# Peilun-Tommy-Li/pHNN-MPC

Hardware: AMD Instinct MI355X
Metric: pHNN-MPC rollouts+grads/sec, cartpole H=50 batch=65536 (higher is better)
Workload: dtype f32

## Files before the change

### phnn_mpc_amd/csrc/phnn_kernels.hip.h

```cpp
#pragma once
#include <hip/hip_runtime.h>

#include <type_traits>

#include "../../include/phnn_mpc.h"

#define DEV __device__ __forceinline__
#ifdef PHNN_CACHED_TAPE
#define PHNN_NT_STORE(v, p) (*(p) = (v))
#define PHNN_NT_LOAD(p) (*(p))
#else
#define PHNN_NT_STORE(v, p) __builtin_nontemporal_store((v), (p))
#define PHNN_NT_LOAD(p) __builtin_nontemporal_load((p))
#endif

using f32x4 = __attribute__((ext_vector_type(4))) float;
using f32x2 = __attribute__((ext_vector_type(2))) float;

constexpr int kTileB = 16;
#ifndef PHNN_KMAXWAVES
#define PHNN_KMAXWAVES 8
#endif
constexpr int kMaxWaves = PHNN_KMAXWAVES;
constexpr int kScrFloats = 16 * 20;

struct Lane {
  int lane, i, q;
  int w;
  float* xch;
};

template <int T>
struct Act {
  f32x4 v[T];
};

DEV f32x4 mfma(float a, float b, f32x4 c) { return __builtin_amdgcn_mfma_f32_16x16x4f32(a, b, c, 0, 0, 0); }

DEV f32x4 splat4(float s) { return f32x4{s, s, s, s}; }

DEV f32x4 fma4(f32x4 a, f32x4 b, f32x4 c) { return __builtin_elementwise_fma(a, b, c); }
DEV f32x4 dtanh(f32x4 a) { return __builtin_elementwise_fma(-a, a, f32x4{1.0f, 1.0f, 1.0f, 1.0f}); }

DEV float sel4(f32x4 v, int q) { return q == 0 ? v[0] : (q == 1 ? v[1] : (q == 2 ? v[2] : v[3])); }

DEV float tanh_scaled(float x, float c) {
  float e = __builtin_amdgcn_exp2f(x * c);
  return __builtin_fmaf(-2.0f, __builtin_amdgcn_rcpf(e + 1.0f), 1.0f);
}

template <bool ACCURATE>
DEV float tanh_dev(float x) {
  if (ACCURATE) {
    float ax = __builtin_fabsf(x);
    float s = x * x;
    float p = -0.007265716325491667f;
    p = __builtin_fmaf(p, s, 0.021598778665065765f);
    p = __builtin_fmaf(p, s, -0.053949106484651566f);
    p = __builtin_fmaf(p, s, 0.13333284854888916f);
    p = __builtin_fmaf(p, s, -0.3333333432674408f);
    float small = __builtin_fmaf(ax * s, p, ax);
    float e = __builtin_amdgcn_exp2f(ax * 2.8853900817779268f);
    float big = __builtin_fmaf(-2.0f, __builtin_amdgcn_rcpf(e + 1.0f), 1.0f);
    float r = ax < 0.4f ? small : big;
    return __builtin_copysignf(r, x);
  }
  float e = __builtin_amdgcn_exp2f(x * 2.8853900817779268f);
  return __builtin_fmaf(-2.0f, __builtin_amdgcn_rcpf(e + 1.0f), 1.0f);
}

DEV void sincos_dev(float x, float& sn, float& cs) {
  float k = __builtin_rintf(x * 0.6366197723675814f);
  float r = __builtin_fmaf(k, -1.5707963705062866f, x);
  r = __builtin_fmaf(k, 4.371138828673793e-08f, r);
  r = __builtin_fmaf(k, 1.7763568394002505e-15f, r);
  float r2 = r * r;
  float p = 2.723737452470232e-06f;
  p = __builtin_fmaf(p, r2, -0.00019839986634906381f);
  p = __builtin_fmaf(p, r2, 0.008333331905305386f);
  p = __builtin_fmaf(p, r2, -0.1666666716337204f);
  float s0 = __builtin_fmaf(r * r2, p, r);
  float q = -2.721424721130461e-07f;
  q = __builtin_fmaf(q, r2, 2.479966133250855e-05f);
  q = __builtin_fmaf(q, r2, -0.0013888884568586946f);
  q = __builtin_fmaf(q, r2, 0.0416666679084301f);
  float c0 = __builtin_fmaf(r2 * r2, q, __builtin_fmaf(-0.5f, r2, 1.0f));
  int n = (int)k;
  float ss = (n & 1) ? c0 : s0;
  float cc = (n & 1) ? s0 : c0;
  sn = (n & 2) ? -ss : ss;
  cs = ((n + 1) & 2) ? -cc : cc;
}

DEV void keep_lds_reads_local() { asm volatile("" ::: "memory"); }

template <int T>
DEV void tanh_act(Act<T>& a) {
  constexpr bool ACCURATE = T <= 4;
#pragma unroll
  for (int t = 0; t < T; ++t)
#pragma unroll
    for (int r = 0; r < 4; ++r) a.v[t][r] = tanh_dev<ACCURATE>(a.v[t][r]);
}

template <int T>
constexpr bool kPreScaled = T > 4;

template <int T>
DEV void tanh_act_pre(Act<T>& a) {
#pragma unroll
  for (int t = 0; t < T; ++t)
#pragma unroll
    for (int r = 0; r < 4; ++r) {
      if (kPreScaled<T>) a.v[t][r] = __builtin_fmaf(-2.0f, __builtin_amdgcn_rcpf(__builtin_amdgcn_exp2f(a.v[t][r]) + 1.0f), 1.0f);
      else a.v[t][r] = tanh_dev<true>(a.v[t][r]);
    }
}

template <int T>
DEV void load_vec(Act<T>& o, const float* vec, Lane ln) {
  keep_lds_reads_local();
#pragma unroll
  for (int t = 0; t < T; ++t) o.v[t] = *reinterpret_cast<const f32x4*>(vec + 16 * t + 4 * ln.q);
}

template <int T>
DEV void zero_act(Act<T>& o) {
#pragma unroll
  for (int t = 0; t < T; ++t) o.v[t] = splat4(0.f);
}

template <int T>
DEV void in_layer(Act<T>& o, const float* Wf, Lane ln, float xk) {
  keep_lds_reads_local();
#pragma unroll
  for (int nt = 0; nt < T; ++nt) o.v[nt] = mfma(Wf[nt * 64 + ln.lane], xk, o.v[nt]);
}

template <int TO, int TI>
DEV void sq_fwd(Act<TO>& o, const float* W, Lane ln, const Act<TI>& in) {
  constexpr int LD = 16 * TI + 4;
  keep_lds_reads_local();
  const float* base = W + ln.i * LD + 4 * ln.q;
  if (TO == 1) {
    f32x4 e = o.v[0], d = splat4(0.f);
#pragma unroll
    for (int t = 0; t < TI; ++t) {
      f32x4 a = *reinterpret_cast<const f32x4*>(base + 16 * t);
      e = mfma(a[0], in.v[t][0], e);
      d = mfma(a[1], in.v[t][1], d);
      e = mfma(a[2], in.v[t][2], e);
      d = mfma(a[3], in.v[t][3], d);
    }
    o.v[0] = e + d;
    return;
  }
  constexpr int G = TO < 4 ? TO : 4;
#pragma unroll
  for (int t = 0; t < TI; ++t) {
#pragma unroll
    for (int n0 = 0; n0 < TO; n0 += G) {
      f32x4 a[G];
#pragma unroll
      for (int g = 0; g < G; ++g) a[g] = *reinterpret_cast<const f32x4*>(base + (n0 + g) * 16 * LD + 16 * t);
#pragma unroll
      for (int r = 0; r < 4; ++r)
#pragma unroll
        for (int g = 0; g < G; ++g) o.v[n0 + g] = mfma(a[g][r], in.v[t][r], o.v[n0 + g]);
    }
  }
}

template <int TO, int TI>
DEV void sq_bwd(Act<TO>& o, const float* W, Lane ln, const Act<TI>& in) {
  constexpr int LD = 16 * TO + 4;
  keep_lds_reads_local();
  const float* base = W + 4 * ln.q * LD + ln.i;
#pragma unroll
  for (int t = 0; t < TI; ++t)
#pragma unroll
    for (int r = 0; r < 4; ++r)
#pragma unroll
      for (int nt = 0; nt < TO; ++nt) o.v[nt] = mfma(base[(16 * t + r) * LD + 16 * nt], in.v[t][r], o.v[nt]);
}

constexpr int MM_F32 = 0, MM_BF16X3 = 1, MM_F16X2 = 2;
using bf16x2 = __attribute__((ext_vector_type(2))) __bf16;
using bf16x4 = __attribute__((ext_vector_type(4))) __bf16;
using bf16x8 = __attribute__((ext_vector_type(8))) __bf16;
using u32x4 = __attribute__((ext_vector_type(4))) unsigned;

DEV f32x4 mfma_bf(bf16x8 a, bf16x8 b, f32x4 c) { return __builtin_amdgcn_mfma_f32_16x16x32_bf16(a, b, c, 0, 0, 0); }

DEV unsigned pk_bf16(float a, float b) {
  f32x2 v = {a, b};
  return __builtin_bit_cast(unsigned, __builtin_convertvector(v, bf16x2));
}

DEV void matrix_phase_begin() {
#if !defined(PHNN_NO_SETPRIO) && !defined(PHNN_STATIC_PRIO)
  __builtin_amdgcn_s_setprio(0);
#endif
}
DEV void matrix_phase_end() {
#if !defined(PHNN_NO_SETPRIO) && !defined(PHNN_STATIC_PRIO)
  __builtin_amdgcn_s_setprio(2);
#endif
}
DEV void static_prio(int wave) {
#ifdef PHNN_STATIC_PRIO
  if (wave >= 4) __builtin_amdgcn_s_setprio(1);
#endif
}

template <int T>
struct Split3 {
  bf16x8 h[T / 2], m[T / 2], l[T / 2];
};

template <int T>
DEV void split_act(const Act<T>& a, Split3<T>& o) {
#pragma unroll
  for (int s = 0; s < T / 2; ++s) {
    u32x4 H, M, Lo;
#pragma unroll
    for (int p = 0; p < 4; ++p) {
      float x0 = a.v[2 * s + (p >> 1)][2 * (p & 1)], x1 = a.v[2 * s + (p >> 1)][2 * (p & 1) + 1];
      unsigned hb = pk_bf16(x0, x1);
      float r0 = x0 - __builtin_bit_cast(float, hb << 16), r1 = x1 - __builtin_bit_cast(float, hb & 0xffff0000u);
      unsigned mb = pk_bf16(r0, r1);
      float t0 = r0 - __builtin_bit_cast(float, mb << 16), t1 = r1 - __builtin_bit_cast(float, mb & 0xffff0000u);
      H[p] = hb;
      M[p] = mb;
      Lo[p] = pk_bf16(t0, t1);
    }
    o.h[s] = __builtin_bit_cast(bf16x8, H);
    o.m[s] = __builtin_bit_cast(bf16x8, M);
    o.l[s] = __builtin_bit_cast(bf16x8, Lo);
  }
}

template <int HID>
struct BfImg {
  static constexpr int RS = HID + 16;
  static constexpr int PART = HID * RS * 2;
  static constexpr int FLOATS = 3 * PART / 4;
};

DEV void mfma6x2(f32x4& o0, f32x4& o1, const bf16x8 (&a)[2][3], bf16x8 xh, bf16x8 xm, bf16x8 xl) {
  o0 = mfma_bf(a[0][2], xh, o0);
  o1 = mfma_bf(a[1][2], xh, o1);
  o0 = mfma_bf(a[0][0], xl, o0);
  o1 = mfma_bf(a[1][0], xl, o1);
  o0 = mfma_bf(a[0][1], xm, o0);
  o1 = mfma_bf(a[1][1], xm, o1);
  o0 = mfma_bf(a[0][1], xh, o0);
  o1 = mfma_bf(a[1][1], xh, o1);
  o0 = mfma_bf(a[0][0], xm, o0);
  o1 = mfma_bf(a[1][0], xm, o1);
  o0 = mfma_bf(a[0][0], xh, o0);
  o1 = mfma_bf(a[1][0], xh, o1);
}

template <int T>
DEV void sq_fwd_bf(Act<T>& o, const float* Wimg, Lane ln, const Split3<T>& in) {
  using I = BfImg<16 * T>;
  keep_lds_reads_local();
  matrix_phase_begin();
  const char* base = reinterpret_cast<const char*>(Wimg) + ln.i * (I::RS * 2) + ln.q * 16;
#ifdef PHNN_PREFETCH_BF
  {
    bf16x8 a[2][2][3];
    auto loadg = [&](int g, bf16x8 (&dst)[2][3]) {
      const int n0 = 2 * (g / (T / 2)), s = g % (T / 2);
#pragma unroll
      for (int gg = 0; gg < 2; ++gg)
#pragma unroll
        for (int p = 0; p < 3; ++p)
          dst[gg][p] = *reinterpret_cast<const bf16x8*>(base + p * I::PART + (n0 + gg) * 16 * (I::RS * 2) + s * 64);
    };
    constexpr int NG = (T / 2) * (T / 2);
    loadg(0, a[0]);
#pragma unroll
    for (int g = 0; g < NG; ++g) {
      if (g + 1 < NG) loadg(g + 1, a[(g + 1) & 1]);
      __builtin_amdgcn_sched_barrier(0);
      const int n0 = 2 * (g / (T / 2)), s = g % (T / 2);
      mfma6x2(o.v[n0], o.v[n0 + 1], a[g & 1], in.h[s], in.m[s], in.l[s]);
      __builtin_amdgcn_sched_barrier(0);
    }
    matrix_phase_end();
    return;
  }
#endif
#pragma unroll
  for (int n0 = 0; n0 < T; n0 += 2) {
#pragma unroll
    for (int s = 0; s < T / 2; ++s) {
      bf16x8 a[2][3];
#pragma unroll
      for (int g = 0; g < 2; ++g)
#pragma unroll
        for (int p = 0; p < 3; ++p)
          a[g][p] = *reinterpret_cast<const bf16x8*>(base + p * I::PART + (n0 + g) * 16 * (I::RS * 2) + s * 64);
      mfma6x2(o.v[n0], o.v[n0 + 1], a, in.h[s], in.m[s], in.l[s]);
    }
  }
  matrix_phase_end();
}

template <int T>
DEV void sq_bwd_bf(Act<T>& o, const float* Wimg, Lane ln, const Split3<T>& in) {
  using I = BfImg<16 * T>;
  keep_lds_reads_local();
  matrix_phase_begin();
  typedef bf16x4 __attribute__((address_space(3))) * lds_bf4;
  typedef char __attribute__((address_space(3))) * lds_cp;
  const int a4 = (ln.lane & 15) >> 2, pp = ln.lane & 3;
  lds_cp base = (lds_cp) const_cast<char*>(reinterpret_cast<const char*>(Wimg)) + (4 * ln.q + a4) * (I::RS * 2) + 16 * pp;
#ifdef PHNN_PREFETCH_BF
  {
    bf16x8 a[2][2][3];
    auto loadg = [&](int g, bf16x8 (&dst)[2][3]) {
      const int n0 = 2 * (g / (T / 2)), s = g % (T / 2);
#pragma unroll
      for (int gg = 0; gg < 2; ++gg) {
        const int nt = n0 + gg;
#pragma unroll
        for (int p = 0; p < 3; ++p) {
          lds_cp off = base + p * I::PART + 32 * s * (I::RS * 2) + (64 * (nt >> 1) + 8 * (nt & 1));
          bf16x4 lo = __builtin_amdgcn_ds_read_tr16_b64_v4bf16((lds_bf4)off);
          bf16x4 hi = __builtin_amdgcn_ds_read_tr16_b64_v4bf16((lds_bf4)(off + 16 * (I::RS * 2)));
          dst[gg][p] = __builtin_shufflevector(lo, hi, 0, 1, 2, 3, 4, 5, 6, 7);
        }
      }
    };
    constexpr int NG = (T / 2) * (T / 2);
    loadg(0, a[0]);
#pragma unroll
    for (int g = 0; g < NG; ++g) {
      if (g + 1 < NG) loadg(g + 1, a[(g + 1) & 1]);
      __builtin_amdgcn_sched_barrier(0);
      const int n0 = 2 * (g / (T / 2)), s = g % (T / 2);
      mfma6x2(o.v[n0], o.v[n0 + 1], a[g & 1], in.h[s], in.m[s], in.l[s]);
      __builtin_amdgcn_sched_barrier(0);
    }
    matrix_phase_end();
    return;
  }
#endif
#pragma unroll
  for (int n0 = 0; n0 < T; n0 += 2) {
#pragma unroll
    for (int s = 0; s < T / 2; ++s) {
      bf16x8 a[2][3];
#pragma unroll
      for (int g = 0; g < 2; ++g) {
        const int nt = n0 + g;
#pragma unroll
        for (int p = 0; p < 3; ++p) {
          lds_cp off = base + p * I::PART + 32 * s * (I::RS * 2) + (64 * (nt >> 1) + 8 * (nt & 1));
          bf16x4 lo = __builtin_amdgcn_ds_read_tr16_b64_v4bf16((lds_bf4)off);
          bf16x4 hi = __builtin_amdgcn_ds_read_tr16_b64_v4bf16((lds_bf4)(off + 16 * (I::RS * 2)));
          a[g][p] = __builtin_shufflevector(lo, hi, 0, 1, 2, 3, 4, 5, 6, 7);
        }
      }
      mfma6x2(o.v[n0], o.v[n0 + 1], a, in.h[s], in.m[s], in.l[s]);
    }
  }
  matrix_phase_end();
}

using f16x2 = __attribute__((ext_vector_type(2))) _Float16;
using f16x4 = __attribute__((ext_vector_type(4))) _Float16;
using f16x8 = __attribute__((ext_vector_type(8))) _Float16;
typedef __fp16 fp16x4_t __attribute__((__vector_size__(4 * sizeof(__fp16))));

DEV f32x4 mfma_h(f16x8 a, f16x8 b, f32x4 c) { return __builtin_amdgcn_mfma_f32_16x16x32_f16(a, b, c, 0, 0, 0); }

DEV f32x2 residual_h(f16x2 h, f32x2 x) {
#ifdef PHNN_NO_FMAMIX
  return x - __builtin_convertvector(h, f32x2);
#endif
  unsigned hb = __builtin_bit_cast(unsigned, h);
  f32x2 r;
  asm("v_fma_mix_f32 %0, %1, -1.0, %2 op_sel_hi:[1,0,0]" : "=v"(r[0]) : "v"(hb), "v"(x[0]));
  asm("v_fma_mix_f32 %0, %1, -1.0, %2 op_sel:[1,0,0] op_sel_hi:[1,0,0]" : "=v"(r[1]) : "v"(hb), "v"(x[1]));
  return r;
}

template <int T>
struct Split2 {
  f16x8 h[T / 2], l[T / 2];
};

template <int T>
DEV void split_act_h(const Act<T>& a, Split2<T>& o) {
#pragma unroll
  for (int s = 0; s < T / 2; ++s) {
    u32x4 H, Lo;
#pragma unroll
    for (int p = 0; p < 4; ++p) {
      f32x2 x = {a.v[2 * s + (p >> 1)][2 * (p & 1)], a.v[2 * s + (p >> 1)][2 * (p & 1) + 1]};
      f16x2 hb = __builtin_convertvector(x, f16x2);
      f32x2 r = residual_h(hb, x);
      H[p] = __builtin_bit_cast(unsigned, hb);
      Lo[p] = __builtin_bit_cast(unsigned, __builtin_convertvector(r, f16x2));
    }
    o.h[s] = __builtin_bit_cast(f16x8, H);
    o.l[s] = __builtin_bit_cast(f16x8, Lo);
  }
}

template <int HID>
struct HfImg {
  static constexpr int RS = HID + 16;
  static constexpr int PART = HID * RS * 2;
  static constexpr int FLOATS = 2 * PART / 4;
};

DEV f16x8 in_frag_h(f32x4 x) {
// ... 250 lines not shown
  u32x4 H = __builtin_bit_cast(u32x4, o.h[P]), Lo = __builtin_bit_cast(u32x4, o.l[P]);
  H[j] = __builtin_bit_cast(unsigned, hb);
  Lo[j] = __builtin_bit_cast(unsigned, __builtin_convertvector(r, f16x2));
  o.h[P] = __builtin_bit_cast(f16x8, H);
  o.l[P] = __builtin_bit_cast(f16x8, Lo);
}
template <int TI>
struct To4Pairs {
  static_assert(TI >= 2 && TI % 2 == 0, "pairs of tiles");
  const float* row;
  f32x4 tot, o0, o1, a;
  DEV To4Pairs(const float* Wt, Lane ln) : row(Wt + (ln.i & 3) * (16 * TI + 8) + 4 * ln.q) {
    a = *reinterpret_cast<const f32x4*>(row);
  }
  DEV void put(int P, int j, float x0, float x1) {
    const int t = 2 * P + (j >> 1), e = 2 * (j & 1);
    if (j == 0) o0 = o1 = splat4(0.f);
    o0 = __builtin_amdgcn_mfma_f32_4x4x1f32(a[e], x0, o0, 0, 0, 0);
    o1 = __builtin_amdgcn_mfma_f32_4x4x1f32(a[e + 1], x1, o1, 0, 0, 0);
    if (e == 2 && t + 1 < TI) a = *reinterpret_cast<const f32x4*>(row + 16 * (t + 1));
    if (j == 3) tot = P == 0 ? o0 + o1 : tot + (o0 + o1);
  }
  DEV f32x4 finish() const { return to4_kslots(tot); }
};

template <int T>
DEV void store_act(float* dst, Lane ln, const Act<T>& a) {
#pragma unroll
  for (int t = 0; t < T; ++t) PHNN_NT_STORE(a.v[t], reinterpret_cast<f32x4*>(dst) + t * 64 + ln.lane);
}
template <int T>
DEV void load_act(const float* src, Lane ln, Act<T>& a) {
#pragma unroll
  for (int t = 0; t < T; ++t) {
#ifdef PHNN_PLAIN_STASH_LOADS
    a.v[t] = reinterpret_cast<const f32x4*>(src)[t * 64 + ln.lane];
#else
    a.v[t] = PHNN_NT_LOAD(reinterpret_cast<const f32x4*>(src) + t * 64 + ln.lane);
#endif
  }
}

constexpr float kFix24 = 8388607.0f;
typedef unsigned u32x3 __attribute__((ext_vector_type(3), aligned(4)));
template <int T>
DEV void store_act24(float* dst, Lane ln, const Act<T>& a) {
#pragma unroll
  for (int t = 0; t < T; ++t) {
    unsigned q[4];
#pragma unroll
    for (int r = 0; r < 4; ++r) q[r] = (unsigned)(int)__builtin_rintf(a.v[t][r] * kFix24);
    u32x3 d = {__builtin_amdgcn_perm(q[1], q[0], 0x04020100u),
               __builtin_amdgcn_perm(q[2], q[1], 0x05040201u),
               __builtin_amdgcn_perm(q[3], q[2], 0x06050402u)};
    PHNN_NT_STORE(d, reinterpret_cast<u32x3*>(reinterpret_cast<char*>(dst) + (t * 64 + ln.lane) * 12));
  }
}
template <int T>
DEV void load_act24(const float* src, Lane ln, Act<T>& a) {
#pragma unroll
  for (int t = 0; t < T; ++t) {
    const u32x3 d = PHNN_NT_LOAD(reinterpret_cast<const u32x3*>(reinterpret_cast<const char*>(src) + (t * 64 + ln.lane) * 12));
    const int q0 = (int)(d[0] << 8) >> 8;
    const int q1 = (int)(__builtin_amdgcn_alignbit(d[1], d[0], 24) << 8) >> 8;
    const int q2 = (int)(__builtin_amdgcn_alignbit(d[2], d[1], 16) << 8) >> 8;
    const int q3 = (int)d[2] >> 8;
    a.v[t] = f32x4{(float)q0, (float)q1, (float)q2, (float)q3} * (1.0f / kFix24);
  }
}

DEV void gather16(float* scr, Lane ln, f32x4 mine, float (&out)[16]) {
  float* row = scr + ln.i * 20;
  *reinterpret_cast<f32x4*>(row + 4 * ln.q) = mine;
  __builtin_amdgcn_wave_barrier();
#pragma unroll
  for (int k = 0; k < 4; ++k) {
    f32x4 v = *reinterpret_cast<const f32x4*>(row + 4 * k);
    out[4 * k + 0] = v[0];
    out[4 * k + 1] = v[1];
    out[4 * k + 2] = v[2];
    out[4 * k + 3] = v[3];
  }
  __builtin_amdgcn_wave_barrier();
}

DEV float reduce_q(float v) {
#ifdef PHNN_BPERMUTE_REDUCE
  v += __shfl_xor(v, 16);
  v += __shfl_xor(v, 32);
  return v;
#else
  float b;
  asm volatile("v_mov_b32 %1, %0\n\ts_nop 1\n\tv_permlane16_swap_b32 %0, %1\n\ts_nop 0" : "+v"(v), "=&v"(b));
  v += b;
  asm volatile("v_mov_b32 %1, %0\n\ts_nop 1\n\tv_permlane32_swap_b32 %0, %1\n\ts_nop 0" : "+v"(v), "=&v"(b));
  return v + b;
#endif
}


template <int HID, int MM = MM_F32>
struct LayH2 {
  static constexpr int T = HID / 16, LD = HID + 4, LR = HID + 8;
  static constexpr int oW2 = 0;
  static constexpr int W2F = MM == MM_F32 ? HID * LD : (MM == MM_BF16X3 ? BfImg<HID>::FLOATS : HfImg<HID>::FLOATS);
  static constexpr int oW1h = oW2 + W2F;
  static constexpr int oW1f = oW1h + (MM == MM_F16X2 ? T * 64 * 4 : 0);
  static constexpr int oB1 = oW1f + T * 64;
  static constexpr int oB2 = oB1 + HID;
  static constexpr int oW3 = oB2 + HID;
  static constexpr int oW3B = oW3 + HID;
  static constexpr int oW3S = oW3B + HID;
  static constexpr int oW1T = oW3S + HID;
  static constexpr int oB3 = oW1T + 4 * LR;
  static constexpr int SIZE = oB3 + 4;
};

template <int HID, int MM = MM_F32>
struct LayH1 {
  static constexpr int T = HID / 16, LD = HID + 4, LR = HID + 8;
  static constexpr bool HF = MM == MM_F16X2;
  static constexpr int RS = HID + 16;
  static constexpr int FPART = 16 * RS * 2;
  static constexpr int BPART = HID * 16 * 2;
  static constexpr int oV2 = 0;
  static constexpr int oV2T = oV2 + 2 * FPART / 4;
  static constexpr int V2F = HF ? (2 * FPART + 2 * BPART) / 4 : 16 * LD;
  static constexpr int oV1h = oV2 + V2F;
  static constexpr int oV1f = oV1h + (HF ? T * 64 * 4 : 0);
  static constexpr int oC1 = oV1f + T * 64;
  static constexpr int oC2 = oC1 + HID;
  static constexpr int oSc = oC2 + 16;
  static constexpr int oV1T = oSc + 4;
  static constexpr int SIZE = oV1T + 4 * LR;
};

constexpr int kRecSmall = 40;
template <int T, int NBIG>
struct WRec {
  static constexpr int VEC = T * 256;
  static constexpr int oSmall = NBIG * VEC;
  static constexpr int SIZE = oSmall + 16 * kRecSmall;
};

#ifdef PHNN_CACHED_RECORDS
#define PHNN_REC_STORE(v, p) (*(p) = (v))
#define PHNN_REC_LOAD(p) (*(p))
#else
#define PHNN_REC_STORE(v, p) __builtin_nontemporal_store((v), (p))
#define PHNN_REC_LOAD(p) __builtin_nontemporal_load((p))
#endif
template <int T>
DEV void store_rec(float* dst, Lane ln, const Act<T>& a) {
#pragma unroll
  for (int t = 0; t < T; ++t) PHNN_REC_STORE(a.v[t], reinterpret_cast<f32x4*>(dst) + t * 64 + ln.lane);
}
template <int T>
DEV void store_rec_scaled(float* dst, Lane ln, const Act<T>& a, float s) {
#pragma unroll
  for (int t = 0; t < T; ++t) PHNN_REC_STORE(a.v[t] * s, reinterpret_cast<f32x4*>(dst) + t * 64 + ln.lane);
}

constexpr int ACT_TANH = 0, ACT_SILU = 2, ACT_RELU = 3, ACT_ELU = 4, ACT_GELU = 5;

DEV float gelu_pdf(float z) { return 0.3989422804014327f * __builtin_amdgcn_exp2f(z * z * -0.7213475204444817f); }
DEV float gelu_cdf(float z) { return __builtin_fmaf(0.5f, erff(z * 0.7071067811865476f), 0.5f); }

template <int ACT>
DEV void act_eval(float z, float& a, float& d1) {
  if (ACT == ACT_RELU) {
    a = fmaxf(z, 0.f);
    d1 = z > 0.f ? 1.0f : 0.0f;
  } else if (ACT == ACT_ELU) {
    a = z > 0.f ? z : expm1f(z);
    d1 = z > 0.f ? 1.0f : __builtin_amdgcn_exp2f(z * 1.4426950408889634f);
  } else if (ACT == ACT_GELU) {
    const float c = gelu_cdf(z);
    a = z * c;
    d1 = __builtin_fmaf(z, gelu_pdf(z), c);
  } else {
    const float s = __builtin_amdgcn_rcpf(1.0f + __builtin_amdgcn_exp2f(z * -1.4426950408889634f));
    a = z * s;
    d1 = __builtin_fmaf(a, 1.0f - s, s);
  }
}
template <int ACT>
DEV float act_d2(float z) {
  if (ACT == ACT_RELU) return 0.0f;
  if (ACT == ACT_ELU) return z > 0.f ? 0.0f : __builtin_amdgcn_exp2f(z * 1.4426950408889634f);
  if (ACT == ACT_GELU) return gelu_pdf(z) * fmaxf(__builtin_fmaf(-z, z, 2.0f), -3.0e38f);
  const float s = __builtin_amdgcn_rcpf(1.0f + __builtin_amdgcn_exp2f(z * -1.4426950408889634f));
  return s * (1.0f - s) * __builtin_fmaf(z, 1.0f - 2.0f * s, 2.0f);
}
template <int ACT, int T>
DEV void act_of(const Act<T>& z, Act<T>& a) {
#pragma unroll
  for (int t = 0; t < T; ++t)
#pragma unroll
    for (int r = 0; r < 4; ++r) {
      float av, d;
      act_eval<ACT>(z.v[t][r], av, d);
      a.v[t][r] = av;
    }
}
template <int ACT, int T>
DEV void mul_d1(Act<T>& g, const Act<T>& z) {
#pragma unroll
  for (int t = 0; t < T; ++t)
#pragma unroll
    for (int r = 0; r < 4; ++r) {
      float a, d;
      act_eval<ACT>(z.v[t][r], a, d);
      g.v[t][r] *= d;
    }
}

constexpr int TAPE_NONE = 0, TAPE_MPC = 1, TAPE_TRAIN = 2;
template <class M, int TK>
constexpr int tape_floats() {
  if constexpr (TK == TAPE_MPC && M::CURV) return M::TAPE_C;
  else return M::STASH;
}

template <int HID>
struct HTape {
  Act<HID / 16> a1, a2, q1;
};

template <int HID, bool WANT_H, int ACT>
DEV f32x4 hnet_grad_g(const float* L, Lane ln, f32x4 x, HTape<HID>& tp, float& Hval) {
  using Y = LayH2<HID, MM_F32>;
  constexpr int T = Y::T;
  load_vec<T>(tp.a1, L + Y::oB1, ln);
  in_layer<T>(tp.a1, L + Y::oW1f, ln, sel4(x, ln.q));
  {
    Act<T> a;
    act_of<ACT, T>(tp.a1, a);
    load_vec<T>(tp.a2, L + Y::oB2, ln);
    sq_fwd<T, T>(tp.a2, L + Y::oW2, ln, a);
  }
  Act<T> g;
  float s = 0.f;
  keep_lds_reads_local();
#pragma unroll
  for (int t = 0; t < T; ++t) {
    f32x4 w3 = *reinterpret_cast<const f32x4*>(L + Y::oW3 + 16 * t + 4 * ln.q);
#pragma unroll
    for (int r = 0; r < 4; ++r) {
      float a, d;
      act_eval<ACT>(tp.a2.v[t][r], a, d);
      if (WANT_H) s = __builtin_fmaf(w3[r], a, s);
      g.v[t][r] = w3[r] * d;
    }
  }
  if (WANT_H) Hval = reduce_q(s) + L[Y::oB3];
  zero_act<T>(tp.q1);
  sq_bwd<T, T>(tp.q1, L + Y::oW2, ln, g);
#pragma unroll
  for (int t = 0; t < T; ++t) g.v[t] = tp.q1.v[t];
  mul_d1<ACT, T>(g, tp.a1);
  return to4_rep<T>(L + Y::oW1T, ln, g);
}
template <int HID, int ACT>
DEV void hnet_layer1_g(const float* L, Lane ln, f32x4 x, Act<HID / 16>& z1) {
  using Y = LayH2<HID, MM_F32>;
  load_vec<Y::T>(z1, L + Y::oB1, ln);
  in_layer<Y::T>(z1, L + Y::oW1f, ln, sel4(x, ln.q));
}
template <int HID, int ACT>
DEV f32x4 hnet_hvp_g(const float* L, Lane ln, HTape<HID>& tp, f32x4 v) {
  using Y = LayH2<HID, MM_F32>;
  constexpr int T = Y::T;
  Act<T> ad1, w;
  zero_act<T>(ad1);
  in_layer<T>(ad1, L + Y::oW1f, ln, sel4(v, ln.q));
#pragma unroll
  for (int t = 0; t < T; ++t)
#pragma unroll
    for (int r = 0; r < 4; ++r) {
      const float z = tp.a1.v[t][r], zd = ad1.v[t][r];
      float a, d;
      act_eval<ACT>(z, a, d);
      tp.q1.v[t][r] = tp.q1.v[t][r] * (act_d2<ACT>(z) * zd);
      ad1.v[t][r] = d * zd;
    }
  zero_act<T>(w);
  sq_fwd<T, T>(w, L + Y::oW2, ln, ad1);
  keep_lds_reads_local();
#pragma unroll
  for (int t = 0; t < T; ++t) {
    f32x4 w3 = *reinterpret_cast<const f32x4*>(L + Y::oW3 + 16 * t + 4 * ln.q);
#pragma unroll
    for (int r = 0; r < 4; ++r) w.v[t][r] = w3[r] * (act_d2<ACT>(tp.a2.v[t][r]) * w.v[t][r]);
  }
  Act<T> qd;
  zero_act<T>(qd);
  sq_bwd<T, T>(qd, L + Y::oW2, ln, w);
  mul_d1<ACT, T>(qd, tp.a1);
#pragma unroll
  for (int t = 0; t < T; ++t) qd.v[t] = qd.v[t] + tp.q1.v[t];
  return to4_rep<T>(L + Y::oW1T, ln, qd);
}

template <int HID, bool WANT_H, int MM = MM_F32, int SITE = kInHFwd, int ACT = ACT_TANH, int FE = 0>
DEV f32x4 hnet_grad(const float* L, Lane ln, f32x4 z, HTape<HID>& tp, float& Hval) {
  if constexpr (ACT != ACT_TANH) {
    static_assert(MM == MM_F32, "SiLU / ReLU run on the all-f32 kernels");
    return hnet_grad_g<HID, WANT_H, ACT>(L, ln, z, tp, Hval);
  }
  using Y = LayH2<HID, MM>;
  constexpr int T = Y::T;
  load_vec<T>(tp.a1, L + Y::oB1, ln);
  in_layer_mm<T, MM, SITE>(tp.a1, L, Y::oW1f, Y::oW1h, ln, z);
  tanh_act_pre<T>(tp.a1);
  load_vec<T>(tp.a2, L + Y::oB2, ln);
  constexpr bool FUSABLE = MM == MM_F16X2 && SITE == kInHFwd && T >= 2 && T % 2 == 0;
  constexpr bool FUSE_ACT = FUSABLE && (FE & kFuseSites & kFuseK1Act) != 0, FUSE_RED = FUSABLE && (FE & kFuseSites & kFuseK1Red) != 0;
  Split2<T> spg{};
  float s = 0.f;
  if constexpr (FUSE_ACT) {
    Split2<T> sp;
    split_act_h<T>(tp.a1, sp);
    const float c = L[Y::oB3 + 1];
    f32x4 w3 = splat4(0.f), w3b = *reinterpret_cast<const f32x4*>(L + Y::oW3B + 4 * ln.q);
    if (WANT_H) w3 = *reinterpret_cast<const f32x4*>(L + Y::oW3 + 4 * ln.q);
    auto act = [&](auto pre) {
      return [&](int P, int j) {
        const int t = 2 * P + (j >> 1), e = 2 * (j & 1);
        f32x2 g;
#pragma unroll
        for (int k = 0; k < 2; ++k) {
          const float x = tp.a2.v[t][e + k];
          const float a = decltype(pre)::value ? __builtin_fmaf(-2.0f, __builtin_amdgcn_rcpf(__builtin_amdgcn_exp2f(x) + 1.0f), 1.0f)
                                               : tanh_scaled(x, c);
          tp.a2.v[t][e + k] = a;
          if (WANT_H) s = __builtin_fmaf(w3[e + k], a, s);
          g[k] = w3b[e + k] * __builtin_fmaf(-a, a, 1.0f);
        }
        if (e == 2 && t + 1 < T) {
          if (WANT_H) w3 = *reinterpret_cast<const f32x4*>(L + Y::oW3 + 16 * (t + 1) + 4 * ln.q);
          w3b = *reinterpret_cast<const f32x4*>(L + Y::oW3B + 16 * (t + 1) + 4 * ln.q);
        }
        split_put_h<T>(spg, P, j, g);
      };
    };
    if (kPreScaled<T> && c == 1.0f) sq_fwd_h<T>(tp.a2, L + Y::oW2, ln, sp, act(std::true_type()));
    else sq_fwd_h<T>(tp.a2, L + Y::oW2, ln, sp, act(std::false_type()));
  } else if (MM == MM_BF16X3) {
    Split3<T> sp;
    split_act<T>(tp.a1, sp);
    sq_fwd_bf<T>(tp.a2, L + Y::oW2, ln, sp);
  } else if (MM == MM_F16X2) {
    Split2<T> sp;
    split_act_h<T>(tp.a1, sp);
    sq_fwd_h<T>(tp.a2, L + Y::oW2, ln, sp);
  } else {
    sq_fwd<T, T>(tp.a2, L + Y::oW2, ln, tp.a1);
  }
  if constexpr (FUSE_ACT) {
  } else if (MM == MM_F16X2 || kPreScaled<T>) {
    const float c = L[Y::oB3 + 1];
    if (kPreScaled<T> && c == 1.0f) {
      tanh_act_pre<T>(tp.a2);
    } else {
#pragma unroll
      for (int t = 0; t < T; ++t)
#pragma unroll
        for (int r = 0; r < 4; ++r) tp.a2.v[t][r] = tanh_scaled(tp.a2.v[t][r], c);
    }
  } else {
    tanh_act<T>(tp.a2);
  }
  Act<T> g;
  keep_lds_reads_local();
  if constexpr (!FUSE_ACT) {
#pragma unroll
    for (int t = 0; t < T; ++t) {
      if (WANT_H) {
        f32x4 w3 = *reinterpret_cast<const f32x4*>(L + Y::oW3 + 16 * t + 4 * ln.q);
#pragma unroll
        for (int r = 0; r < 4; ++r) s = __builtin_fmaf(w3[r], tp.a2.v[t][r], s);
      }
      f32x4 w3b = *reinterpret_cast<const f32x4*>(L + Y::oW3B + 16 * t + 4 * ln.q);
      g.v[t] = w3b * dtanh(tp.a2.v[t]);
    }
  }
  if (WANT_H) Hval = reduce_q(s) + L[Y::oB3];
  zero_act<T>(tp.q1);
  if constexpr (FUSABLE) {
    if constexpr (!FUSE_ACT) split_act_h<T>(g, spg);
    if constexpr (FUSE_RED) {
      To4Pairs<T> red(L + Y::oW1T, ln);
      sq_bwd_h<T>(tp.q1, L + Y::oW2, ln, spg, [&](int P, int j) {
        const int t = 2 * P + (j >> 1), e = 2 * (j & 1);
        const float a0 = tp.a1.v[t][e], a1 = tp.a1.v[t][e + 1];
        red.put(P, j, tp.q1.v[t][e] * __builtin_fmaf(-a0, a0, 1.0f), tp.q1.v[t][e + 1] * __builtin_fmaf(-a1, a1, 1.0f));
      });
      return red.finish();
    } else {
      sq_bwd_h<T>(tp.q1, L + Y::oW2, ln, spg);
    }
  } else if (MM == MM_BF16X3) {
    Split3<T> sp;
    split_act<T>(g, sp);
    sq_bwd_bf<T>(tp.q1, L + Y::oW2, ln, sp);
  } else if (MM == MM_F16X2) {
    Split2<T> sp;
    split_act_h<T>(g, sp);
    sq_bwd_h<T>(tp.q1, L + Y::oW2, ln, sp);
  } else {
    sq_bwd<T, T>(tp.q1, L + Y::oW2, ln, g);
  }
#pragma unroll
  for (int t = 0; t < T; ++t) g.v[t] = tp.q1.v[t] * dtanh(tp.a1.v[t]);
  return to4_rep<T>(L + Y::oW1T, ln, g);
}

template <int HID, int MM, int ACT = ACT_TANH>
DEV void hnet_layer1(const float* L, Lane ln, f32x4 z, Act<HID / 16>& a1) {
  if constexpr (ACT != ACT_TANH) return hnet_layer1_g<HID, ACT>(L, ln, z, a1);
  using Y = LayH2<HID, MM>;
  load_vec<Y::T>(a1, L + Y::oB1, ln);
  in_layer_mm<Y::T, MM, kInHRecomp>(a1, L, Y::oW1f, Y::oW1h, ln, z);
  tanh_act_pre<Y::T>(a1);
}

template <int HID>
struct CurvImg {
  static constexpr int RS = HID + 16, PART = 10 * RS * 2;
  static constexpr int oConst = 2 * PART / 4;
  static constexpr int FLOATS = oConst + 4;
};
struct Curv {
  float m[16];
};
template <int T>
DEV void hnet_curv_operand(const Act<T>& q1, const Act<T>& a1, Split2<T>& sp) {
  Act<T> c;
#pragma unroll
  for (int t = 0; t < T; ++t) c.v[t] = (q1.v[t] * dtanh(a1.v[t])) * a1.v[t];
  split_act_h<T>(c, sp);
}
template <int HID>
DEV f32x4 hnet_curv_kstep(const float* P, Lane ln, int s, f16x8 ch, f16x8 cl) {
  using I = CurvImg<HID>;
  keep_lds_reads_local();
  const int a = ln.i >> 2, b = ln.i & 3, lo = a < b ? a : b, hi = a < b ? b : a;
  const int row = (lo * (9 - lo)) / 2 + (hi - lo);
  const char* base = reinterpret_cast<const char*>(P) + row * (I::RS * 2) + ln.q * 16 + s * 64;
  const f16x8 ah = *reinterpret_cast<const f16x8*>(base);
  const f16x8 al = *reinterpret_cast<const f16x8*>(base + I::PART);
  return mfma_h(ah, ch, mfma_h(ah, cl, mfma_h(al, ch, splat4(0.f))));
}
template <int HID>
DEV f32x4 hnet_curv(const float* P, Lane ln, const HTape<HID>& tp) {
  constexpr int T = HID / 16;
  Split2<T> sp;
  hnet_curv_operand<T>(tp.q1, tp.a1, sp);
  f32x4 tot = hnet_curv_kstep<HID>(P, ln, 0, sp.h[0], sp.l[0]);
#pragma unroll
  for (int s = 1; s < T / 2; ++s) tot = tot + hnet_curv_kstep<HID>(P, ln, s, sp.h[s], sp.l[s]);
  return tot * P[CurvImg<HID>::oConst];
}
DEV void spread_curv(f32x4 mine, Lane ln, Curv& c) {
#pragma unroll
  for (int r = 0; r < 4; ++r)
#pragma unroll
    for (int j = 0; j < 4; ++j) c.m[4 * r + j] = __shfl(mine[j], 16 * r + ln.i);
}
DEV f32x4 curv_apply(const Curv& c, f32x4 v) {
  f32x4 o;
#pragma unroll
  for (int r = 0; r < 4; ++r) {
    float s = 0.f;
#pragma unroll
    for (int j = 0; j < 4; ++j) s = __builtin_fmaf(c.m[4 * r + j], v[j], s);
    o[r] = s;
  }
  return o;
}

template <int HID, bool COMPACT>
DEV void hnet_tape_store(float* stash, int oC, const float* P, Lane ln, const HTape<HID>& tp, f32x4 dH) {
  constexpr int T = HID / 16;
  store_act<T>(stash, ln, tp.a2);
  if constexpr (COMPACT) {
    if (ln.q == 0) PHNN_NT_STORE(dH, reinterpret_cast<f32x4*>(stash + T * 256) + ln.i);
    PHNN_NT_STORE(hnet_curv<HID>(P, ln, tp), reinterpret_cast<f32x4*>(stash + oC) + ln.i * 4 + ln.q);
  } else {
    store_act<T>(stash + T * 256, ln, tp.q1);
    if (ln.q == 0) PHNN_NT_STORE(dH, reinterpret_cast<f32x4*>(stash + 2 * T * 256) + ln.i);
  }
}
template <int T, bool COMPACT>
DEV f32x4 tape_load_dH(const float* stash, Lane ln) {
  return PHNN_NT_LOAD(reinterpret_cast<const f32x4*>(stash + (COMPACT ? 1 : 2) * T * 256) + ln.i);
}
DEV void load_curv(const float* src, Lane ln, Curv& c) {
  const f32x4* p = reinterpret_cast<const f32x4*>(src) + ln.i * 4;
#pragma unroll
  for (int k = 0; k < 4; ++k) {
    f32x4 v = PHNN_NT_LOAD(p + k);
#pragma unroll
    for (int e = 0; e < 4; ++e) c.m[4 * k + e] = v[e];
  }
}
template <int HID, bool COMPACT>
DEV void hnet_tape_load(const float* stash, int oC, Lane ln, HTape<HID>& tp, Curv& cv) {
  constexpr int T = HID / 16;
  load_act<T>(stash, ln, tp.a2);
  if constexpr (COMPACT) load_curv(stash + oC, ln, cv);
  else load_act<T>(stash + T * 256, ln, tp.q1);
}

template <int HID, int MM = MM_F32, bool WG = false, int ACT = ACT_TANH, int SITE = kInHHvp, bool CQ = false, int FE = 0>
DEV f32x4 hnet_hvp(const float* L, Lane ln, HTape<HID>& tp, f32x4 v, float* rec = nullptr, const Curv* cv = nullptr) {
  static_assert(!CQ || (MM == MM_F16X2 && ACT == ACT_TANH && !WG), "the curvature block exists for f16x2 Tanh MPC kernels");
  if constexpr (ACT != ACT_TANH) {
    static_assert(!WG, "weight-gradient kernels exist for Tanh models only");
    return hnet_hvp_g<HID, ACT>(L, ln, tp, v);
  }
  using Y = LayH2<HID, MM>;
  constexpr int T = Y::T;
  float unscale = 1.0f;
  if (MM == MM_F16X2) {
    float mx = fmaxf(fmaxf(__builtin_fabsf(v[0]), __builtin_fabsf(v[1])), fmaxf(__builtin_fabsf(v[2]), __builtin_fabsf(v[3])));
    int e = 0;
    (void)__builtin_frexpf(mx, &e);
    e = (mx > 0.f && mx < 3.0e38f) ? e : 0;
    v = v * __builtin_ldexpf(1.0f, -e);
    unscale = __builtin_ldexpf(1.0f, e);
  }
  Act<T> ad1, w;
  zero_act<T>(ad1);
  in_layer_mm<T, MM, SITE>(ad1, L, Y::oW1f, Y::oW1h, ln, v);
#pragma unroll
  for (int t = 0; t < T; ++t) ad1.v[t] = dtanh(tp.a1.v[t]) * ad1.v[t];
  if constexpr (!CQ) {
#pragma unroll
    for (int t = 0; t < T; ++t) tp.q1.v[t] = tp.q1.v[t] * (tp.a1.v[t] * ad1.v[t]);
  }
  zero_act<T>(w);
  constexpr bool FUSABLE = CQ && T >= 2 && T % 2 == 0;
  constexpr bool FUSE_ACT = FUSABLE && (FE & kFuseSites & kFuseK2Act) != 0, FUSE_RED = FUSABLE && (FE & kFuseSites & kFuseK2Red) != 0;
  Split2<T> spw{};
  if constexpr (FUSE_ACT) {
    Split2<T> sp;
    split_act_h<T>(ad1, sp);
    f32x4 w3 = *reinterpret_cast<const f32x4*>(L + Y::oW3S + 4 * ln.q);
    sq_fwd_h<T>(w, L + Y::oW2, ln, sp, [&](int P, int j) {
      const int t = 2 * P + (j >> 1), e = 2 * (j & 1);
      f32x2 x;
#pragma unroll
      for (int k = 0; k < 2; ++k) {
        const float a2 = tp.a2.v[t][e + k];
        const float ad2 = __builtin_fmaf(-a2, a2, 1.0f) * w.v[t][e + k];
        x[k] = w3[e + k] * (a2 * ad2);
      }
      if (e == 2 && t + 1 < T) w3 = *reinterpret_cast<const f32x4*>(L + Y::oW3S + 16 * (t + 1) + 4 * ln.q);
      split_put_h<T>(spw, P, j, x);
    });
  } else {
    if (MM == MM_BF16X3) {
      Split3<T> sp;
      split_act<T>(ad1, sp);
      sq_fwd_bf<T>(w, L + Y::oW2, ln, sp);
    } else if (MM == MM_F16X2) {
      Split2<T> sp;
      split_act_h<T>(ad1, sp);
      sq_fwd_h<T>(w, L + Y::oW2, ln, sp);
    } else {
      sq_fwd<T, T>(w, L + Y::oW2, ln, ad1);
    }
    keep_lds_reads_local();
#pragma unroll
    for (int t = 0; t < T; ++t) {
      f32x4 w3 = *reinterpret_cast<const f32x4*>(L + Y::oW3S + 16 * t + 4 * ln.q);
      f32x4 a2 = tp.a2.v[t];
      f32x4 ad2 = dtanh(a2) * w.v[t];
      if (WG) PHNN_REC_STORE(ad2 * unscale, reinterpret_cast<f32x4*>(rec + 2 * T * 256) + t * 64 + ln.lane);
      w.v[t] = w3 * (a2 * ad2);
    }
  }
  Act<T> qd;
  zero_act<T>(qd);
  if constexpr (FUSABLE) {
    if constexpr (!FUSE_ACT) split_act_h<T>(w, spw);
    if constexpr (FUSE_RED) {
      To4Pairs<T> red(L + Y::oW1T, ln);
      sq_bwd_h<T>(qd, L + Y::oW2, ln, spw, [&](int P, int j) {
        const int t = 2 * P + (j >> 1), e = 2 * (j & 1);
        const float a0 = tp.a1.v[t][e], a1 = tp.a1.v[t][e + 1];
        red.put(P, j, qd.v[t][e] * __builtin_fmaf(-a0, a0, 1.0f), qd.v[t][e + 1] * __builtin_fmaf(-a1, a1, 1.0f));
      });
      return (red.finish() * (-2.0f * L[Y::oB3 + 2]) + curv_apply(*cv, v)) * unscale;
    } else {
      sq_bwd_h<T>(qd, L + Y::oW2, ln, spw);
    }
  } else if (MM == MM_BF16X3) {
    Split3<T> sp;
    split_act<T>(w, sp);
    sq_bwd_bf<T>(qd, L + Y::oW2, ln, sp);
  } else if (MM == MM_F16X2) {
    Split2<T> sp;
    split_act_h<T>(w, sp);
    sq_bwd_h<T>(qd, L + Y::oW2, ln, sp);
  } else {
    sq_bwd<T, T>(qd, L + Y::oW2, ln, w);
  }
  if (WG) store_rec_scaled<T>(rec + 3 * T * 256, ln, qd, unscale);
#pragma unroll
  for (int t = 0; t < T; ++t) {
    if constexpr (CQ) qd.v[t] = qd.v[t] * dtanh(tp.a1.v[t]);
    else qd.v[t] = __builtin_elementwise_fma(qd.v[t], dtanh(tp.a1.v[t]), tp.q1.v[t]);
  }
  f32x4 Hv = to4_rep<T>(L + Y::oW1T, ln, qd);
  if constexpr (CQ) return (Hv * (-2.0f * L[Y::oB3 + 2]) + curv_apply(*cv, v)) * unscale;
  return Hv * (-2.0f * unscale * L[Y::oB3 + 2]);
}

template <int HID, int MM>
DEV f32x4 h1_out_hf(const float* L, Lane ln, const Split2<HID / 16>& sp) {
  using Y = LayH1<HID, MM>;
  constexpr int T = Y::T;
  keep_lds_reads_local();
  const char* base = reinterpret_cast<const char*>(L + Y::oV2) + ln.i * (Y::RS * 2) + ln.q * 16;
  f32x4 o0 = splat4(0.f), o1 = splat4(0.f), o2 = splat4(0.f);
#pragma unroll
  for (int s = 0; s < T / 2; ++s) {
    f16x8 ah = *reinterpret_cast<const f16x8*>(base + s * 64);
    f16x8 al = *reinterpret_cast<const f16x8*>(base + Y::FPART + s * 64);
    o0 = mfma_h(al, sp.h[s], o0);
    o1 = mfma_h(ah, sp.l[s], o1);
    o2 = mfma_h(ah, sp.h[s], o2);
  }
  const float inv = L[Y::oSc];
  f32x4 c2 = *reinterpret_cast<const f32x4*>(L + Y::oC2 + 4 * ln.q);
  return ((o0 + o1) + o2) * inv + c2;
}

template <int HID, int MM>
DEV void h1_bwd_operands(const float* L, Lane ln, const float (&obar)[16], f16x8& b1, f16x8& b2, float& unscale) {
  using Y = LayH1<HID, MM>;
  float mx = 0.f;
#pragma unroll
  for (int k = 0; k < 16; ++k) mx = fmaxf(mx, __builtin_fabsf(obar[k]));
  int e = 0;
  (void)__builtin_frexpf(mx, &e);
  e = (mx > 0.f && mx < 3.0e38f) ? e : 0;
  const float sc = __builtin_ldexpf(1.0f, -e);
  unscale = __builtin_ldexpf(1.0f, e) * L[Y::oSc];
  const bool second = (ln.q & 1) != 0, lo_half = ln.q >= 2;
  u32x4 B1, B2;
#pragma unroll
  for (int p = 0; p < 4; ++p) {
    f32x2 v = {(second ? obar[8 + 2 * p] : obar[2 * p]) * sc, (second ? obar[9 + 2 * p] : obar[2 * p + 1]) * sc};
    f16x2 hb2 = __builtin_convertvector(v, f16x2);
    f32x2 r = residual_h(hb2, v);
    unsigned hbits = __builtin_bit_cast(unsigned, hb2), lbits = __builtin_bit_cast(unsigned, __builtin_convertvector(r, f16x2));
    B1[p] = lo_half ? lbits : hbits;
    B2[p] = lo_half ? 0u : hbits;
  }
  b1 = __builtin_bit_cast(f16x8, B1);
  b2 = __builtin_bit_cast(f16x8, B2);
}

DEV void store_rf(float* dst, Lane ln, f32x4 o) {
  if (ln.w == 0) PHNN_NT_STORE(o, reinterpret_cast<f32x4*>(dst) + ln.i * 4 + ln.q);
}
DEV void load_rf(const float* src, Lane ln, float (&rf)[16]) {
  const f32x4* p = reinterpret_cast<const f32x4*>(src) + ln.i * 4;
#pragma unroll
  for (int k = 0; k < 4; ++k) {
    f32x4 v = PHNN_NT_LOAD(p + k);
#pragma unroll
    for (int e = 0; e < 4; ++e) rf[4 * k + e] = v[e];
  }
}
template <int HID, int MM = MM_F32, int SITE = kInHNet1, int ACT = ACT_TANH>
DEV void h1_hidden(const float* L, Lane ln, f32x4 x, Act<HID / 16>& h) {
  using Y = LayH1<HID, MM>;
  constexpr int T = Y::T;
  load_vec<T>(h, L + Y::oC1, ln);
  in_layer_mm<T, MM, SITE>(h, L, Y::oV1f, Y::oV1h, ln, x);
  if constexpr (ACT == ACT_TANH) tanh_act_pre<T>(h);
}

template <int HID, int MM = MM_F32, int SITE = kInHNet1, int ACT = ACT_TANH>
DEV void h1_fwd(const float* L, float* scr, Lane ln, f32x4 x, Act<HID / 16>& h, float (&out)[16], float* rf_stash = nullptr) {
  using Y = LayH1<HID, MM>;
  constexpr int T = Y::T;
  load_vec<T>(h, L + Y::oC1, ln);
  in_layer_mm<T, MM, SITE>(h, L, Y::oV1f, Y::oV1h, ln, x);
  if constexpr (ACT != ACT_TANH) {
    static_assert(MM == MM_F32, "SiLU / ReLU run on the all-f32 kernels");
    Act<T> a;
    act_of<ACT, T>(h, a);
    Act<1> og;
    og.v[0] = *reinterpret_cast<const f32x4*>(L + Y::oC2 + 4 * ln.q);
    sq_fwd<1, T>(og, L + Y::oV2, ln, a);
    if (rf_stash) store_rf(rf_stash, ln, og.v[0]);
    gather16(scr, ln, og.v[0], out);
    return;
  }
  tanh_act_pre<T>(h);
  Act<1> o;
  if (Y::HF) {
    Split2<T> sp;
    split_act_h<T>(h, sp);
    o.v[0] = h1_out_hf<HID, MM>(L, ln, sp);
  } else {
    o.v[0] = *reinterpret_cast<const f32x4*>(L + Y::oC2 + 4 * ln.q);
    sq_fwd<1, T>(o, L + Y::oV2, ln, h);
  }
  if (rf_stash) store_rf(rf_stash, ln, o.v[0]);
  gather16(scr, ln, o.v[0], out);
}

template <int HID, int MM = MM_F32, bool WG = false, int ACT = ACT_TANH>
DEV f32x4 h1_bwd(const float* L, Lane ln, const Act<HID / 16>& h, const float (&obar)[16], float* rec = nullptr) {
  using Y = LayH1<HID, MM>;
  constexpr int T = Y::T;
  Act<T> hb;
  if constexpr (ACT != ACT_TANH) {
    static_assert(MM == MM_F32 && !WG, "SiLU / ReLU: all-f32 kernels, no weight-gradient records");
    Act<1> ob;
#pragma unroll
    for (int r = 0; r < 4; ++r)
      ob.v[0][r] = ln.q == 0 ? obar[r] : (ln.q == 1 ? obar[4 + r] : (ln.q == 2 ? obar[8 + r] : obar[12 + r]));
    zero_act<T>(hb);
    sq_bwd<T, 1>(hb, L + Y::oV2, ln, ob);
    mul_d1<ACT, T>(hb, h);
    return to4_rep<T>(L + Y::oV1T, ln, hb);
  }
  float unscale = 1.0f;
  if (Y::HF) {
    f16x8 b1, b2;
    h1_bwd_operands<HID, MM>(L, ln, obar, b1, b2, unscale);
    keep_lds_reads_local();
    const char* base = reinterpret_cast<const char*>(L + Y::oV2T) + ln.i * 32 + (ln.q & 1) * 16;
#pragma unroll
    for (int nt = 0; nt < T; ++nt) {
      f16x8 ah = *reinterpret_cast<const f16x8*>(base + nt * 512);
      f16x8 al = *reinterpret_cast<const f16x8*>(base + Y::BPART + nt * 512);
      hb.v[nt] = mfma_h(ah, b1, mfma_h(al, b2, splat4(0.f)));
    }
  } else {
    Act<1> ob;
#pragma unroll
    for (int r = 0; r < 4; ++r)
      ob.v[0][r] = ln.q == 0 ? obar[r] : (ln.q == 1 ? obar[4 + r] : (ln.q == 2 ? obar[8 + r] : obar[12 + r]));
    zero_act<T>(hb);
    sq_bwd<T, 1>(hb, L + Y::oV2, ln, ob);
  }
#pragma unroll
  for (int t = 0; t < T; ++t) hb.v[t] = hb.v[t] * dtanh(h.v[t]);
  if (WG) store_rec_scaled<T>(rec, ln, hb, Y::HF ? unscale : 1.0f);
  f32x4 xb = to4_rep<T>(L + Y::oV1T, ln, hb);
  return Y::HF ? xb * unscale : xb;
}

template <int N>
DEV void sym_from_rf(const float (&rf)[16], float (&S)[N][N]) {
#pragma unroll
  for (int i = 0; i < N; ++i) {
    S[i][i] = rf[i * N + i];
#pragma unroll
    for (int j = i + 1; j < N; ++j) S[i][j] = S[j][i] = (rf[i * N + j] + rf[j * N + i]) * 0.5f;
  }
}
template <int N>
DEV void rbar_from(f32x4 lam, f32x4 dH, const float (&Stl)[N], const float (&StdH)[N], float (&rbar)[16]) {
  float m[N][N];
#pragma unroll
  for (int k = 0; k < 16; ++k) rbar[k] = 0.f;
#pragma unroll
  for (int i = 0; i < N; ++i)
#pragma unroll
    for (int j = 0; j < N; ++j) m[i][j] = __builtin_fmaf(lam[i], StdH[j], dH[i] * Stl[j]);
#pragma unroll
  for (int i = 0; i < N; ++i) {
    rbar[i * N + i] = -m[i][i];
#pragma unroll
    for (int j = i + 1; j < N; ++j) rbar[i * N + j] = rbar[j * N + i] = (m[i][j] + m[j][i]) * -0.5f;
  }
}

template <int N_, int HID_, bool FIXG_, int MM_ = MM_F32, int MI_ = 1, int ACT_ = ACT_TANH>
struct PhnnModel {
  static constexpr int N = N_, HID = HID_, T = HID / 16, MM = MM_, MI = MI_, ACT = ACT_;
  static constexpr bool FIXG = FIXG_, SPLIT = false;
  static_assert(N_ * MI_ <= 16 && MI_ <= 4, "G_net output n*m <= 16, m <= 4");
  static constexpr int SCR = kScrFloats;
  static constexpr int oH = 0;
  static constexpr int oR = oH + LayH2<HID, MM>::SIZE;
  static constexpr int oGn = oR + LayH1<HID, MM>::SIZE;
  static constexpr int oJ = oGn + (FIXG ? 0 : LayH1<HID, MM>::SIZE);
  static constexpr int oG = oJ + 16;
  static constexpr int oP = oG + 16;
  static constexpr bool CURV = MM == MM_F16X2 && ACT == ACT_TANH &&
                               4 * (oP + CurvImg<HID>::FLOATS + kMaxWaves * SCR) <= 160 * 1024;
  static constexpr int IMG = oP + (CURV ? CurvImg<HID>::FLOATS : 0);
  static constexpr int FUSE = (HID_ != 128 || !FIXG_) ? 0 : ((MI_ <= 2 ? PHNN_FUSE_K1 : 0) | (MI_ == 1 ? PHNN_FUSE_K2 : 0));

  static constexpr int oStashRf = 2 * T * 256 + 64;
  static constexpr int STASH = oStashRf + 256;
  static constexpr int oTapeRf = T * 256 + 64, oTapeC = oTapeRf + 256, TAPE_C = oTapeC + 256;

  template <bool WANT_H, int TK = TAPE_NONE, int FE = 0>
  DEV static f32x4 f(const float* L, float* scr, Lane ln, f32x4 x, f32x4 u, float& Hval, float* stash = nullptr) {
    constexpr bool ST = TK != TAPE_NONE, CT = TK == TAPE_MPC && CURV;
    keep_lds_reads_local();
    HTape<HID> tp;
    f32x4 dH = hnet_grad<HID, WANT_H, MM, kInHFwd, ACT, FE>(L + oH, ln, x, tp, Hval);
    if (ST) hnet_tape_store<HID, CT>(stash, oTapeC, L + oP, ln, tp, dH);
    Act<T> hR;
    float rf[16];
    h1_fwd<HID, MM, kInHNet1, ACT>(L + oR, scr, ln, x, hR, rf, ST ? stash + (CT ? oTapeRf : oStashRf) : nullptr);
    float G[N * MI];
    if (FIXG) {
#pragma unroll
      for (int i = 0; i < N * MI; ++i) G[i] = L[oG + i];
    } else {
      Act<T> hG;
      float gf[16];
      h1_fwd<HID, MM, kInHNet1, ACT>(L + oGn, scr, ln, x, hG, gf);
#pragma unroll
      for (int i = 0; i < N * MI; ++i) G[i] = gf[i];
    }
    return combine(L, rf, dH, G, u);
  }

  DEV static f32x4 combine(const float* L, const float (&rf)[16], f32x4 dH, const float (&G)[N * MI], f32x4 u) {
    float S[N][N], StdH[N];
    sym_from_rf<N>(rf, S);
#pragma unroll
    for (int k = 0; k < N; ++k) {
      float a = 0.f;
#pragma unroll
      for (int i = 0; i < N; ++i) a = __builtin_fmaf(S[i][k], dH[i], a);
      StdH[k] = a;
    }
    f32x4 dx = splat4(0.f);
#pragma unroll
    for (int i = 0; i < N; ++i) {
      float acc = 0.f;
#pragma unroll
      for (int j = 0; j < N; ++j) acc = __builtin_fmaf(L[oJ + i * N + j], dH[j], acc);
#pragma unroll
      for (int k = 0; k < N; ++k) acc = __builtin_fmaf(-S[i][k], StdH[k], acc);
      if (MI == 1) {
        dx[i] = __builtin_fmaf(G[i], u[0], acc);
      } else {
        float gu = 0.f;
#pragma unroll
        for (int k = 0; k < MI; ++k) gu = __builtin_fmaf(G[i * MI + k], u[k], gu);
        dx[i] = acc + gu;
      }
    }
    return dx;
  }

  static constexpr bool RECHB = !LayH1<HID, MM>::HF;
  static constexpr int NBIG = 4 + (RECHB ? (FIXG ? 1 : 2) : 0);
  using Rec = WRec<T, NBIG>;

  template <bool ST = false, bool WG = false, int INH = -1, int FE = 0>
  DEV static void vjp(const float* L, float* scr, Lane ln, f32x4 x, f32x4 u, f32x4 lam, f32x4& xbar, f32x4& ubar,
                      const float* stash = nullptr, float* rec = nullptr, float Hbar = 0.f) {
    constexpr bool CQ = CURV && !WG;
    keep_lds_reads_local();
    HTape<HID> tp;
    Curv cv;
    float Hdummy;
    f32x4 dH;
    float rf[16];
    if (ST) {
      dH = tape_load_dH<T, CQ>(stash, ln);
      load_rf(stash + (CQ ? oTapeRf : oStashRf), ln, rf);
      hnet_tape_load<HID, CQ>(stash, oTapeC, ln, tp, cv);
    } else {
      dH = hnet_grad<HID, false, MM, INH & kInHRecomp, ACT>(L + oH, ln, x, tp, Hdummy);
      if constexpr (CQ) spread_curv(hnet_curv<HID>(L + oP, ln, tp), ln, cv);
    }
    if (WG && !ST) {
      store_rec<T>(rec, ln, tp.a2);
      store_rec<T>(rec + Rec::VEC, ln, tp.q1);
    }
    f32x4 xb = splat4(0.f);
    float S[N][N], Stl[N], StdH[N];
    {
      Act<T> hR;
      if (ST) {
        h1_hidden<HID, MM, INH & kInHNet1Adj, ACT>(L + oR, ln, x, hR);
      } else {
        h1_fwd<HID, MM, INH & kInHNet1Adj, ACT>(L + oR, scr, ln, x, hR, rf);
      }
      sym_from_rf<N>(rf, S);
#pragma unroll
      for (int k = 0; k < N; ++k) {
        float a = 0.f, c = 0.f;
#pragma unroll
        for (int i = 0; i < N; ++i) {
          a = __builtin_fmaf(S[i][k], lam[i], a);
          c = __builtin_fmaf(S[i][k], dH[i], c);
        }
        Stl[k] = a;
        StdH[k] = c;
      }
      float rbar[16];
      rbar_from<N>(lam, dH, Stl, StdH, rbar);
      xb += h1_bwd<HID, MM, WG && RECHB, ACT>(L + oR, ln, hR, rbar, WG && RECHB ? rec + 4 * Rec::VEC : nullptr);
      if (WG && ln.q == 0) {
        f32x4* sm = reinterpret_cast<f32x4*>(rec + Rec::oSmall + ln.i * kRecSmall);
#pragma unroll
        for (int k = 0; k < 4; ++k) sm[4 + k] = f32x4{rbar[4 * k], rbar[4 * k + 1], rbar[4 * k + 2], rbar[4 * k + 3]};
      }
    }
    ubar = splat4(0.f);
    if (FIXG) {
#pragma unroll
      for (int k = 0; k < MI; ++k)
#pragma unroll
        for (int i = 0; i < N; ++i) ubar[k] = __builtin_fmaf(L[oG + i * MI + k], lam[i], ubar[k]);
    } else {
      Act<T> hG;
      float gf[16], gbar[16];
      h1_fwd<HID, MM, INH & kInHNet1Adj, ACT>(L + oGn, scr, ln, x, hG, gf);
#pragma unroll
      for (int k = 0; k < 16; ++k) gbar[k] = 0.f;
#pragma unroll
      for (int i = 0; i < N; ++i)
#pragma unroll
        for (int k = 0; k < MI; ++k) {
          ubar[k] = __builtin_fmaf(gf[i * MI + k], lam[i], ubar[k]);
          gbar[i * MI + k] = lam[i] * u[k];
        }
      xb += h1_bwd<HID, MM, WG && RECHB, ACT>(L + oGn, ln, hG, gbar, WG && RECHB ? rec + 5 * Rec::VEC : nullptr);
    }
    f32x4 v = splat4(0.f);
#pragma unroll
    for (int j = 0; j < N; ++j) {
      float acc = 0.f;
#pragma unroll
      for (int i = 0; i < N; ++i) acc = __builtin_fmaf(L[oJ + i * N + j], lam[i], acc);
#pragma unroll
      for (int k = 0; k < N; ++k) acc = __builtin_fmaf(-S[j][k], Stl[k], acc);
      v[j] = acc;
    }
    if (WG && ln.q == 0) {
      f32x4* sm = reinterpret_cast<f32x4*>(rec + Rec::oSmall + ln.i * kRecSmall);
      sm[0] = x;
      sm[1] = v;
      sm[2] = lam;
      sm[3] = dH;
      sm[8] = u;
      sm[9] = f32x4{Hbar, 0.f, 0.f, 0.f};
    }
    if (ST) hnet_layer1<HID, MM, ACT>(L + oH, ln, x, tp.a1);
    xbar = xb + hnet_hvp<HID, MM, WG, ACT, INH & kInHHvp, CQ, ST ? FE : 0>(L + oH, ln, tp, v, rec, &cv);
    if (WG) xbar = xbar + Hbar * dH;
  }
};

struct LayM {
  static constexpr int HID = 64, T = 4, LD = HID + 4, LR = HID + 8;
  static constexpr int oW1f = 0;
  static constexpr int oB1 = oW1f + T * 64;
  static constexpr int oW2 = oB1 + HID;
  static constexpr int oB2 = oW2 + HID * LD;
  static constexpr int oWo = oB2 + HID;
  static constexpr int oBo = oWo + 4 * LR;
  static constexpr int oWoTf = oBo + 4;
  static constexpr int oW1T = oWoTf + T * 64;
  static constexpr int SIZE = oW1T + 4 * LR;
};

struct MTape {
  Act<4> a1, a2;
  f32x4 o;
};

DEV void mnet_fwd(const float* L, Lane ln, f32x4 q, MTape& tp) {
  using Y = LayM;
  keep_lds_reads_local();
  load_vec<4>(tp.a1, L + Y::oB1, ln);
  in_layer<4>(tp.a1, L + Y::oW1f, ln, sel4(q, ln.q));
  tanh_act<4>(tp.a1);
  load_vec<4>(tp.a2, L + Y::oB2, ln);
  sq_fwd<4, 4>(tp.a2, L + Y::oW2, ln, tp.a1);
  tanh_act<4>(tp.a2);
  tp.o = to4_rep<4>(L + Y::oWo, ln, tp.a2) + *reinterpret_cast<const f32x4*>(L + Y::oBo);
}

DEV f32x4 mnet_bwd(const float* L, Lane ln, const MTape& tp, f32x4 ob) {
  using Y = LayM;
  keep_lds_reads_local();
  Act<4> d, e;
  zero_act<4>(d);
  in_layer<4>(d, L + Y::oWoTf, ln, sel4(ob, ln.q));
#pragma unroll
  for (int t = 0; t < 4; ++t) d.v[t] = d.v[t] * dtanh(tp.a2.v[t]);
  zero_act<4>(e);
  sq_bwd<4, 4>(e, L + Y::oW2, ln, d);
#pragma unroll
  for (int t = 0; t < 4; ++t) e.v[t] = e.v[t] * dtanh(tp.a1.v[t]);
  return to4_rep<4>(L + Y::oW1T, ln, e);
}

DEV float softplus_dev(float x) { return x > 20.f ? x : log1pf(expf(x)); }
DEV float sigmoid_sp_dev(float x) { return x > 20.f ? 1.0f : 1.0f / (1.0f + expf(-x)); }

constexpr int MASS_CARTPOLE = 0, MASS_CONSTANT = 1, MASS_DIAGONAL = 2, MASS_FULL = 3;

template <int MT>
DEV void mass_from_outputs(f32x4 o, float (&m)[3], float (&w)[3]) {
  if (MT == MASS_DIAGONAL) {
    m[0] = expf(o[0]) + 1e-3f;
    m[2] = expf(o[1]) + 1e-3f;
    m[1] = 0.f;
    w[0] = 1.0f / m[0];
    w[2] = 1.0f / m[2];
    w[1] = 0.f;
  } else {
    const float l00 = softplus_dev(o[0]) + 1e-3f, l10 = o[1], l11 = softplus_dev(o[2]) + 1e-3f;
    m[0] = l00 * l00;
    m[1] = l00 * l10;
    m[2] = l10 * l10 + l11 * l11;
    const float det = m[0] * m[2] - m[1] * m[1];
    w[0] = m[2] / det;
    w[1] = -m[1] / det;
    w[2] = m[0] / det;
  }
}

template <int MT>
DEV f32x4 mass_outputs_bar(f32x4 o, const float (&Mb)[4]) {
  if (MT == MASS_DIAGONAL) return f32x4{Mb[0] * expf(o[0]), Mb[3] * expf(o[1]), 0.f, 0.f};
  const float l00 = softplus_dev(o[0]) + 1e-3f, l10 = o[1], l11 = softplus_dev(o[2]) + 1e-3f;
  const float s00 = 2.0f * Mb[0], s01 = Mb[1] + Mb[2], s11 = 2.0f * Mb[3];
  return f32x4{(s00 * l00 + s01 * l10) * sigmoid_sp_dev(o[0]), s01 * l00 + s11 * l10, (s11 * l11) * sigmoid_sp_dev(o[2]), 0.f};
}

template <int HID_, int MM_ = MM_F32, int MI_ = 1, int MT_ = MASS_CARTPOLE, int ACT_ = ACT_TANH>
struct CanonModel {
  static constexpr int N = 4, HID = HID_, T = HID / 16, MM = MM_, MI = MI_, MT = MT_, ACT = ACT_;
  static constexpr bool SPLIT = false;
  static constexpr int SCR = 0;
  static constexpr int oH = 0;
  static constexpr int oC = oH + LayH2<HID, MM>::SIZE;
  static constexpr int oCG = oC + 12;
  static constexpr int oCW = oC + 28;
  static constexpr int oMn = oC + 32;
  static constexpr int oP = oMn + (MT_ >= MASS_DIAGONAL ? LayM::SIZE : 0);
  static constexpr bool CURV = MM_ == MM_F16X2 && ACT_ == ACT_TANH;
  static constexpr int FUSE = (HID_ == 128 && MT_ <= MASS_CONSTANT) ? PHNN_FUSE_K1 : 0;
  static constexpr int IMG = oP + (CURV ? CurvImg<HID>::FLOATS : 0);

  DEV static void mass_eval(const float* L, Lane ln, f32x4 y, float (&m)[3], float (&w)[3], MTape& mt) {
    if (MT == MASS_CONSTANT) {
      m[0] = L[oC + 0]; m[1] = L[oC + 1]; m[2] = L[oC + 2];
      w[0] = L[oCW + 0]; w[1] = L[oCW + 1]; w[2] = L[oCW + 2];
    } else {
      mnet_fwd(L + oMn, ln, f32x4{y[0], y[1], 0.f, 0.f}, mt);
      mass_from_outputs<MT>(mt.o, m, w);
    }
  }

  DEV static float Base_Gu(const float* L, int row, f32x4 u) {
    float s = 0.f;
#pragma unroll
    for (int k = 0; k < MI; ++k) s = __builtin_fmaf(L[oCG + row * MI + k], u[k], s);
    return s;
  }
  DEV static f32x4 Base_Gt(const float* L, float dpb0, float dpb1) {
    f32x4 ub = splat4(0.f);
#pragma unroll
    for (int k = 0; k < MI; ++k) ub[k] = L[oCG + 2 * MI + k] * dpb0 + L[oCG + 3 * MI + k] * dpb1;
    return ub;
  }

  static constexpr int STASH = 2 * T * 256 + 64;
  static constexpr int oTapeC = T * 256 + 64, TAPE_C = oTapeC + 256;

  template <bool WANT_H, int TK = TAPE_NONE, int FE = 0>
  DEV static f32x4 f(const float* L, float* scr, Lane ln, f32x4 y, f32x4 u, float& Hval, float* stash = nullptr) {
    constexpr bool ST = TK != TAPE_NONE, CT = TK == TAPE_MPC && CURV;
    keep_lds_reads_local();
    if constexpr (MT != MASS_CARTPOLE) {
      float m[3], w[3];
      MTape mt;
      mass_eval(L, ln, y, m, w, mt);
      f32x4 z = {y[0], y[1], m[0] * y[2] + m[1] * y[3], m[1] * y[2] + m[2] * y[3]};
      HTape<HID> tp;
      f32x4 dH = hnet_grad<HID, WANT_H, MM, kInHFwd, ACT, FE>(L + oH, ln, z, tp, Hval);
      if (ST) hnet_tape_store<HID, CT>(stash, oTapeC, L + oP, ln, tp, dH);
      float dp0 = (-dH[0] - L[oC + 6] * dH[2]) + Base_Gu(L, 2, u);
      float dp1 = (-dH[1] - L[oC + 7] * dH[3]) + Base_Gu(L, 3, u);
      return f32x4{w[0] * z[2] + w[1] * z[3], w[1] * z[2] + w[2] * z[3], w[0] * dp0 + w[1] * dp1, w[1] * dp0 + w[2] * dp1};
    }
    float a = L[oC + 0], b = L[oC + 1], c = L[oC + 2];
    float sn, cs;
    sincos_dev(y[1], sn, cs);
    float bc = b * cs;
    f32x4 z = {y[0], y[1], a * y[2] + bc * y[3], bc * y[2] + c * y[3]};
    HTape<HID> tp;
    f32x4 dH = hnet_grad<HID, WANT_H, MM, kInHFwd, ACT, FE>(L + oH, ln, z, tp, Hval);
    if (ST) hnet_tape_store<HID, CT>(stash, oTapeC, L + oP, ln, tp, dH);
    float dp0 = (-dH[0] - L[oC + 6] * dH[2]) + Base_Gu(L, 2, u);
    float dp1 = (-dH[1] - L[oC + 7] * dH[3]) + Base_Gu(L, 3, u);
    float det = (a * c - bc * bc) + 1e-6f;
    float mi00 = c / det, mi01 = -bc / det, mi11 = a / det;
    return f32x4{mi00 * z[2] + mi01 * z[3], mi01 * z[2] + mi11 * z[3], mi00 * dp0 + mi01 * dp1,
                 mi01 * dp0 + mi11 * dp1};
  }

  static constexpr int NBIG = 4;
  using Rec = WRec<T, NBIG>;

  template <bool ST = false, bool WG = false, int INH = -1, int FE = 0>
  DEV static void vjp(const float* L, float* scr, Lane ln, f32x4 y, f32x4 u, f32x4 lam, f32x4& ybar, f32x4& ubar,
                      const float* stash = nullptr, float* rec = nullptr, float Hbar = 0.f) {
    constexpr bool CQ = CURV && !WG;
    Curv cv;
    keep_lds_reads_local();
    if constexpr (MT != MASS_CARTPOLE) {
      float m[3], w[3];
      MTape mt;
      mass_eval(L, ln, y, m, w, mt);
      f32x4 z = {y[0], y[1], m[0] * y[2] + m[1] * y[3], m[1] * y[2] + m[2] * y[3]};
      HTape<HID> tp;
      float Hdummy;
      f32x4 dH;
      if (ST) {
        dH = tape_load_dH<T, CQ>(stash, ln);
        hnet_tape_load<HID, CQ>(stash, oTapeC, ln, tp, cv);
        hnet_layer1<HID, MM, ACT>(L + oH, ln, z, tp.a1);
      } else {
        dH = hnet_grad<HID, false, MM, INH & kInHRecomp, ACT>(L + oH, ln, z, tp, Hdummy);
        if constexpr (CQ) spread_curv(hnet_curv<HID>(L + oP, ln, tp), ln, cv);
      }
      const float Rd2 = L[oC + 6], Rd3 = L[oC + 7];
      const float dp0 = (-dH[0] - Rd2 * dH[2]) + Base_Gu(L, 2, u);
      const float dp1 = (-dH[1] - Rd3 * dH[3]) + Base_Gu(L, 3, u);
      const float pb0 = lam[0] * w[0] + lam[1] * w[1], pb1 = lam[0] * w[1] + lam[1] * w[2];
      const float dpb0 = lam[2] * w[0] + lam[3] * w[1], dpb1 = lam[2] * w[1] + lam[3] * w[2];
      f32x4 v = {-dpb0, -dpb1, -Rd2 * dpb0, -Rd3 * dpb1};
      ubar = Base_Gt(L, dpb0, dpb1);
      if (WG) {
        if (!ST) {
          store_rec<T>(rec, ln, tp.a2);
          store_rec<T>(rec + Rec::VEC, ln, tp.q1);
        }
        if (ln.q == 0) {
          f32x4* sm = reinterpret_cast<f32x4*>(rec + Rec::oSmall + ln.i * kRecSmall);
          sm[0] = z;
          sm[1] = v;
          sm[2] = lam;
          sm[3] = dH;
          sm[4] = f32x4{0.f, 0.f, -dpb0 * dH[2], -dpb1 * dH[3]};
          sm[8] = u;
          sm[9] = f32x4{Hbar, 0.f, 0.f, 0.f};
        }
      }
      f32x4 zb = hnet_hvp<HID, MM, WG, ACT, INH & kInHHvp, CQ, ST ? FE : 0>(L + oH, ln, tp, v, rec, &cv);
      if (WG) zb = zb + Hbar * dH;
      zb[2] += pb0;
      zb[3] += pb1;
      ybar = f32x4{zb[0], zb[1], zb[2] * m[0] + zb[3] * m[1], zb[2] * m[1] + zb[3] * m[2]};
      if (MT >= MASS_DIAGONAL || WG) {
        const float W4[4] = {w[0], w[1], w[1], w[2]};
        const float Wb[4] = {lam[0] * z[2] + lam[2] * dp0, lam[0] * z[3] + lam[2] * dp1,
                             lam[1] * z[2] + lam[3] * dp0, lam[1] * z[3] + lam[3] * dp1};
        float Tm[4], Um[4], Mb[4];
        Tm[0] = W4[0] * Wb[0] + W4[1] * Wb[2]; Tm[1] = W4[0] * Wb[1] + W4[1] * Wb[3];
        Tm[2] = W4[2] * Wb[0] + W4[3] * Wb[2]; Tm[3] = W4[2] * Wb[1] + W4[3] * Wb[3];
        Um[0] = Tm[0] * W4[0] + Tm[1] * W4[2]; Um[1] = Tm[0] * W4[1] + Tm[1] * W4[3];
        Um[2] = Tm[2] * W4[0] + Tm[3] * W4[2]; Um[3] = Tm[2] * W4[1] + Tm[3] * W4[3];
        Mb[0] = zb[2] * y[2] - Um[0];
        Mb[1] = zb[2] * y[3] - Um[1];
        Mb[2] = zb[3] * y[2] - Um[2];
        Mb[3] = zb[3] * y[3] - Um[3];
        if (WG && ln.q == 0) {
          f32x4* sm = reinterpret_cast<f32x4*>(rec + Rec::oSmall + ln.i * kRecSmall);
          sm[5] = f32x4{Mb[0], Mb[1], Mb[2], Mb[3]};
          sm[6] = f32x4{y[0], y[1], 0.f, 0.f};
        }
        if (MT >= MASS_DIAGONAL) {
          f32x4 qb = mnet_bwd(L + oMn, ln, mt, mass_outputs_bar<MT>(mt.o, Mb));
          ybar[0] += qb[0];
          ybar[1] += qb[1];
        }
      }
      return;
    }
    float a = L[oC + 0], b = L[oC + 1], c = L[oC + 2];
    float sn, cs;
    sincos_dev(y[1], sn, cs);
    float bc = b * cs;
    f32x4 z = {y[0], y[1], a * y[2] + bc * y[3], bc * y[2] + c * y[3]};
    HTape<HID> tp;
    float Hdummy;
    f32x4 dH;
    if (ST) {
      dH = tape_load_dH<T, CQ>(stash, ln);
      hnet_tape_load<HID, CQ>(stash, oTapeC, ln, tp, cv);
      hnet_layer1<HID, MM, ACT>(L + oH, ln, z, tp.a1);
    } else {
      dH = hnet_grad<HID, false, MM, INH & kInHRecomp, ACT>(L + oH, ln, z, tp, Hdummy);
      if constexpr (CQ) spread_curv(hnet_curv<HID>(L + oP, ln, tp), ln, cv);
    }
    float Rd2 = L[oC + 6], Rd3 = L[oC + 7];
    float dp0 = (-dH[0] - Rd2 * dH[2]) + Base_Gu(L, 2, u);
    float dp1 = (-dH[1] - Rd3 * dH[3]) + Base_Gu(L, 3, u);
    float det = (a * c - bc * bc) + 1e-6f;
    float rdet = 1.0f / det;
    float mi00 = c * rdet, mi01 = -bc * rdet, mi11 = a * rdet;
    float pb0 = lam[0] * mi00 + lam[1] * mi01, pb1 = lam[0] * mi01 + lam[1] * mi11;
    float dpb0 = lam[2] * mi00 + lam[3] * mi01, dpb1 = lam[2] * mi01 + lam[3] * mi11;
    float mb00 = lam[0] * z[2] + lam[2] * dp0;
    float mb01 = lam[0] * z[3] + lam[1] * z[2] + lam[2] * dp1 + lam[3] * dp0;
    float mb11 = lam[1] * z[3] + lam[3] * dp1;
    f32x4 v = {-dpb0, -dpb1, -Rd2 * dpb0, -Rd3 * dpb1};
    ubar = Base_Gt(L, dpb0, dpb1);
    if (WG) {
      if (!ST) {
        store_rec<T>(rec, ln, tp.a2);
        store_rec<T>(rec + Rec::VEC, ln, tp.q1);
      }
      if (ln.q == 0) {
        f32x4* sm = reinterpret_cast<f32x4*>(rec + Rec::oSmall + ln.i * kRecSmall);
        sm[0] = z;
        sm[1] = v;
        sm[2] = lam;
        sm[3] = dH;
        sm[4] = f32x4{0.f, 0.f, -dpb0 * dH[2], -dpb1 * dH[3]};
        sm[8] = u;
        sm[9] = f32x4{Hbar, 0.f, 0.f, 0.f};
      }
    }
    f32x4 zb = hnet_hvp<HID, MM, WG, ACT, INH & kInHHvp, CQ, ST ? FE : 0>(L + oH, ln, tp, v, rec, &cv);
    if (WG) zb = zb + Hbar * dH;
    zb[2] += pb0;
    zb[3] += pb1;
    float bcb = zb[2] * y[3] + zb[3] * y[2];
    float detb = (-(mb00 * c + mb11 * a) + mb01 * bc) * (rdet * rdet);
    bcb += -mb01 * rdet;
    bcb += -2.0f * bc * detb;
    ybar = f32x4{zb[0], zb[1] + bcb * (-b * sn), zb[2] * a + zb[3] * bc, zb[2] * bc + zb[3] * c};
  }
};

constexpr int kXR0 = 0, kXR1 = 2048, kXR2 = 4096, kXP0 = 6144, kXP1 = 7168, kXchFloats = 8192;
using ActW = Act<2>;

DEV void xch_put(float* region, Lane ln, const Split2<2>& sp) {
  f16x8* p = reinterpret_cast<f16x8*>(region);
  p[ln.w * 64 + ln.lane] = sp.h[0];
  p[(4 + ln.w) * 64 + ln.lane] = sp.l[0];
}
DEV void xch_get(const float* region, Lane ln, Split2<8>& o) {
  const f16x8* p = reinterpret_cast<const f16x8*>(region);
#pragma unroll
  for (int s = 0; s < 4; ++s) {
    o.h[s] = p[s * 64 + ln.lane];
    o.l[s] = p[(4 + s) * 64 + ln.lane];
  }
}
DEV void xch_put_partial(float* set, Lane ln, f32x4 v) { reinterpret_cast<f32x4*>(set)[ln.w * 64 + ln.lane] = v; }
DEV f32x4 xch_sum_partials(const float* set, Lane ln) {
  const f32x4* p = reinterpret_cast<const f32x4*>(set) + ln.lane;
  return to4_kslots(((p[0] + p[64]) + p[128]) + p[192]);
}

DEV void tanh_pre_w(ActW& a) {
#pragma unroll
  for (int t = 0; t < 2; ++t)
#pragma unroll
    for (int r = 0; r < 4; ++r) a.v[t][r] = __builtin_fmaf(-2.0f, __builtin_amdgcn_rcpf(__builtin_amdgcn_exp2f(a.v[t][r]) + 1.0f), 1.0f);
}

DEV void sq_fwd_h_w(ActW& o, const float* Wimg, Lane ln, const Split2<8>& in) {
  using I = HfImg<128>;
  keep_lds_reads_local();
  matrix_phase_begin();
  const char* base = reinterpret_cast<const char*>(Wimg) + ln.i * (I::RS * 2) + ln.q * 16 + (2 * ln.w) * 16 * (I::RS * 2);
#pragma unroll
  for (int s = 0; s < 4; ++s) {
    f16x8 a[2][2];
#pragma unroll
    for (int g = 0; g < 2; ++g)
#pragma unroll
      for (int p = 0; p < 2; ++p) a[g][p] = *reinterpret_cast<const f16x8*>(base + p * I::PART + g * 16 * (I::RS * 2) + s * 64);
    mfma3x2(o.v[0], o.v[1], a, in.h[s], in.l[s]);
  }
  matrix_phase_end();
}

DEV void sq_bwd_h_w(ActW& o, const float* Wimg, Lane ln, const Split2<8>& in) {
  using I = HfImg<128>;
  keep_lds_reads_local();
  matrix_phase_begin();
  typedef fp16x4_t __attribute__((address_space(3))) * lds_h4;
  typedef char __attribute__((address_space(3))) * lds_cp;
  const int a4 = (ln.lane & 15) >> 2, pp = ln.lane & 3;
  lds_cp base = (lds_cp) const_cast<char*>(reinterpret_cast<const char*>(Wimg)) + (4 * ln.q + a4) * (I::RS * 2) + 16 * pp + 64 * ln.w;
#pragma unroll
  for (int s = 0; s < 4; ++s) {
    f16x8 a[2][2];
#pragma unroll
    for (int g = 0; g < 2; ++g)
#pragma unroll
      for (int p = 0; p < 2; ++p) {
        lds_cp off = base + p * I::PART + 32 * s * (I::RS * 2) + 8 * g;
        f16x4 lo = __builtin_bit_cast(f16x4, __builtin_amdgcn_ds_read_tr16_b64_v4f16((lds_h4)off));
        f16x4 hi = __builtin_bit_cast(f16x4, __builtin_amdgcn_ds_read_tr16_b64_v4f16((lds_h4)(off + 16 * (I::RS * 2))));
        a[g][p] = __builtin_shufflevector(lo, hi, 0, 1, 2, 3, 4, 5, 6, 7);
      }
    mfma3x2(o.v[0], o.v[1], a, in.h[s], in.l[s]);
  }
  matrix_phase_end();
}

struct HTapeW {
  ActW a1, a2, q1;
};
DEV void curv_put_w(const float* P, Lane ln, const HTapeW& tp) {
  Split2<2> sp;
  hnet_curv_operand<2>(tp.q1, tp.a1, sp);
  xch_put_partial(ln.xch + kXP1, ln, hnet_curv_kstep<128>(P, ln, ln.w, sp.h[0], sp.l[0]));
}
DEV f32x4 curv_get_w(const float* P, Lane ln) {
  const f32x4* p = reinterpret_cast<const f32x4*>(ln.xch + kXP1) + ln.lane;
  return (((p[0] + p[64]) + p[128]) + p[192]) * P[CurvImg<128>::oConst];
}

template <int SITE = kInHFwd, class PreBarrier>
DEV f32x4 hnet_grad_w(const float* L, Lane ln, f32x4 z, HTapeW& tp, PreBarrier pre_barrier) {
  using Y = LayH2<128, MM_F16X2>;
  const int t0 = 2 * ln.w;
  load_vec<2>(tp.a1, L + Y::oB1 + 16 * t0, ln);
  in_layer_mm<2, MM_F16X2, SITE>(tp.a1, L, Y::oW1f, Y::oW1h, ln, z, t0);
  tanh_pre_w(tp.a1);
  {
    Split2<2> sp;
    split_act_h<2>(tp.a1, sp);
    xch_put(ln.xch + kXR0, ln, sp);
  }
  pre_barrier();
  __syncthreads();
  {
    Split2<8> all;
    xch_get(ln.xch + kXR0, ln, all);
    load_vec<2>(tp.a2, L + Y::oB2 + 16 * t0, ln);
    sq_fwd_h_w(tp.a2, L + Y::oW2, ln, all);
  }
  const float c = L[Y::oB3 + 1];
  if (c == 1.0f) {
    tanh_pre_w(tp.a2);
  } else {
#pragma unroll
    for (int t = 0; t < 2; ++t)
#pragma unroll
      for (int r = 0; r < 4; ++r) tp.a2.v[t][r] = tanh_scaled(tp.a2.v[t][r], c);
  }
  ActW g;
  keep_lds_reads_local();
#pragma unroll
  for (int t = 0; t < 2; ++t) {
    f32x4 w3b = *reinterpret_cast<const f32x4*>(L + Y::oW3B + 16 * (t0 + t) + 4 * ln.q);
    g.v[t] = w3b * dtanh(tp.a2.v[t]);
  }
  {
    Split2<2> sp;
    split_act_h<2>(g, sp);
    xch_put(ln.xch + kXR1, ln, sp);
  }
  __syncthreads();
  {
    Split2<8> all;
    xch_get(ln.xch + kXR1, ln, all);
    zero_act<2>(tp.q1);
    sq_bwd_h_w(tp.q1, L + Y::oW2, ln, all);
  }
#pragma unroll
  for (int t = 0; t < 2; ++t) g.v[t] = tp.q1.v[t] * dtanh(tp.a1.v[t]);
  keep_lds_reads_local();
  return to4_group<2>(L + Y::oW1T + (ln.i & 3) * Y::LR + 16 * t0, ln, g.v);
}

DEV f32x4 hnet_hvp_w(const float* L, Lane ln, HTapeW& tp, f32x4 v, float& scale, float& unscale, f32x4& vn) {
  using Y = LayH2<128, MM_F16X2>;
  const int t0 = 2 * ln.w;
  float mx = fmaxf(fmaxf(__builtin_fabsf(v[0]), __builtin_fabsf(v[1])), fmaxf(__builtin_fabsf(v[2]), __builtin_fabsf(v[3])));
  int e = 0;
  (void)__builtin_frexpf(mx, &e);
  e = (mx > 0.f && mx < 3.0e38f) ? e : 0;
  v = v * __builtin_ldexpf(1.0f, -e);
  vn = v;
  unscale = __builtin_ldexpf(1.0f, e);
  ActW ad1, w;
  zero_act<2>(ad1);
  in_layer_mm<2, MM_F16X2, kInHHvp>(ad1, L, Y::oW1f, Y::oW1h, ln, v, t0);
#pragma unroll
  for (int t = 0; t < 2; ++t) ad1.v[t] = dtanh(tp.a1.v[t]) * ad1.v[t];
  {
    Split2<2> sp;
    split_act_h<2>(ad1, sp);
    xch_put(ln.xch + kXR0, ln, sp);
  }
  __syncthreads();
  {
    Split2<8> all;
    xch_get(ln.xch + kXR0, ln, all);
    zero_act<2>(w);
    sq_fwd_h_w(w, L + Y::oW2, ln, all);
  }
  keep_lds_reads_local();
#pragma unroll
  for (int t = 0; t < 2; ++t) {
    f32x4 w3 = *reinterpret_cast<const f32x4*>(L + Y::oW3S + 16 * (t0 + t) + 4 * ln.q);
    f32x4 a2 = tp.a2.v[t];
    f32x4 ad2 = dtanh(a2) * w.v[t];
    w.v[t] = w3 * (a2 * ad2);
  }
  {
    Split2<2> sp;
    split_act_h<2>(w, sp);
    xch_put(ln.xch + kXR1, ln, sp);
  }
  __syncthreads();
  ActW qd;
  {
    Split2<8> all;
    xch_get(ln.xch + kXR1, ln, all);
    zero_act<2>(qd);
    sq_bwd_h_w(qd, L + Y::oW2, ln, all);
  }
#pragma unroll
  for (int t = 0; t < 2; ++t) qd.v[t] = qd.v[t] * dtanh(tp.a1.v[t]);
  scale = -2.0f * L[Y::oB3 + 2];
  keep_lds_reads_local();
  return to4_group<2>(L + Y::oW1T + (ln.i & 3) * Y::LR + 16 * t0, ln, qd.v);
}

template <int N_>
struct PhnnSplit {
  using Base = PhnnModel<N_, 128, true, MM_F16X2>;
  static constexpr int N = N_, HID = 128, T = 8, MM = MM_F16X2;
  static constexpr bool FIXG = true, SPLIT = true;
  static constexpr int SCR = Base::SCR, IMG = Base::IMG, STASH = Base::STASH, TAPE_C = Base::TAPE_C, MI = 1;
  static constexpr bool CURV = true;
  static constexpr int oH = Base::oH, oR = Base::oR, oJ = Base::oJ, oG = Base::oG;
  using YR = LayH1<128, MM_F16X2>;

  template <int SITE = kInHNet1>
  DEV static void rnet_hidden(const float* L, Lane ln, f32x4 x, ActW& hR) {
    const int t0 = 2 * ln.w;
    load_vec<2>(hR, L + oR + YR::oC1 + 16 * t0, ln);
    in_layer_mm<2, MM_F16X2, SITE>(hR, L + oR, YR::oV1f, YR::oV1h, ln, x, t0);
    tanh_pre_w(hR);
  }
  template <int SITE = kInHNet1>
  DEV static void rnet_layer1(const float* L, Lane ln, f32x4 x, ActW& hR) {
    rnet_hidden<SITE>(L, ln, x, hR);
    Split2<2> sp;
    split_act_h<2>(hR, sp);
    xch_put(ln.xch + kXR2, ln, sp);
  }
  DEV static void rnet_out(const float* L, float* scr, Lane ln, float (&rf)[16], float* rf_stash = nullptr) {
    Split2<8> all;
    xch_get(ln.xch + kXR2, ln, all);
    f32x4 o = h1_out_hf<128, MM_F16X2>(L + oR, ln, all);
    if (rf_stash) store_rf(rf_stash, ln, o);
    gather16(scr, ln, o, rf);
  }

  template <bool WANT_H, int TK = TAPE_NONE, int FE = 0>
  DEV static f32x4 f(const float* L, float* scr, Lane ln, f32x4 x, f32x4 u, float& Hval, float* stash = nullptr) {
    static_assert(!WANT_H, "the split-tile kernels are rollout kernels");
    constexpr bool ST = TK != TAPE_NONE, CT = TK == TAPE_MPC;
    keep_lds_reads_local();
    HTapeW tp;
    ActW hR;
    f32x4 P = hnet_grad_w(L + oH, ln, x, tp, [&]() { rnet_layer1(L, ln, x, hR); });
    xch_put_partial(ln.xch + kXP0, ln, P);
    if (CT) curv_put_w(L + Base::oP, ln, tp);
    float rf[16];
    rnet_out(L, scr, ln, rf, ST ? stash + (CT ? Base::oTapeRf : Base::oStashRf) : nullptr);
    if (ST) {
      store_act<2>(stash + 2 * ln.w * 256, ln, tp.a2);
      if (!CT) store_act<2>(stash + T * 256 + 2 * ln.w * 256, ln, tp.q1);
    }
    __syncthreads();
    f32x4 dH = xch_sum_partials(ln.xch + kXP0, ln);
    if (ST && ln.q == 0 && ln.w == 0) PHNN_NT_STORE(dH, reinterpret_cast<f32x4*>(stash + (CT ? 1 : 2) * T * 256) + ln.i);
    if (CT) store_rf(stash + Base::oTapeC, ln, curv_get_w(L + Base::oP, ln));
    float G[N];
#pragma unroll
    for (int i = 0; i < N; ++i) G[i] = L[oG + i];
    return Base::combine(L, rf, dH, G, u);
  }

  template <bool ST = false, bool WG = false, int INH = -1, int FE = 0>
  DEV static void vjp(const float* L, float* scr, Lane ln, f32x4 x, f32x4 u, f32x4 lam, f32x4& xbar, f32x4& ubar,
                      const float* stash = nullptr, float* rec = nullptr, float Hbar = 0.f) {
    static_assert(!WG, "weight-gradient records come from the whole-tile kernels");
    keep_lds_reads_local();
    const int t0 = 2 * ln.w;
    HTapeW tp;
    ActW hR;
    Curv cv;
    f32x4 dH;
    float rf[16];
    if (ST) {
      dH = tape_load_dH<T, true>(stash, ln);
      load_rf(stash + Base::oTapeRf, ln, rf);
      load_act<2>(stash + t0 * 256, ln, tp.a2);
      load_curv(stash + Base::oTapeC, ln, cv);
      using Y = LayH2<128, MM_F16X2>;
      load_vec<2>(tp.a1, L + oH + Y::oB1 + 16 * t0, ln);
      in_layer_mm<2, MM_F16X2, kInHRecomp>(tp.a1, L + oH, Y::oW1f, Y::oW1h, ln, x, t0);
      tanh_pre_w(tp.a1);
      rnet_hidden<kInHNet1Adj>(L, ln, x, hR);
    } else {
      f32x4 P = hnet_grad_w<kInHRecomp>(L + oH, ln, x, tp, [&]() { rnet_layer1<kInHNet1Adj>(L, ln, x, hR); });
      xch_put_partial(ln.xch + kXP0, ln, P);
      curv_put_w(L + Base::oP, ln, tp);
      rnet_out(L, scr, ln, rf);
      __syncthreads();
      dH = xch_sum_partials(ln.xch + kXP0, ln);
      spread_curv(curv_get_w(L + Base::oP, ln), ln, cv);
    }
    float S[N][N], Stl[N], StdH[N];
    sym_from_rf<N>(rf, S);
#pragma unroll
    for (int k = 0; k < N; ++k) {
      float a = 0.f, c = 0.f;
#pragma unroll
      for (int i = 0; i < N; ++i) {
        a = __builtin_fmaf(S[i][k], lam[i], a);
        c = __builtin_fmaf(S[i][k], dH[i], c);
      }
      Stl[k] = a;
      StdH[k] = c;
    }
    float rbar[16];
    rbar_from<N>(lam, dH, Stl, StdH, rbar);
    float unscaleR;
    f32x4 PR;
    {
      f16x8 b1, b2;
      h1_bwd_operands<128, MM_F16X2>(L + oR, ln, rbar, b1, b2, unscaleR);
      keep_lds_reads_local();
      const char* base = reinterpret_cast<const char*>(L + oR + YR::oV2T) + ln.i * 32 + (ln.q & 1) * 16;
      ActW hb;
#pragma unroll
      for (int t = 0; t < 2; ++t) {
        f16x8 ah = *reinterpret_cast<const f16x8*>(base + (t0 + t) * 512);
        f16x8 al = *reinterpret_cast<const f16x8*>(base + YR::BPART + (t0 + t) * 512);
        hb.v[t] = mfma_h(ah, b1, mfma_h(al, b2, splat4(0.f)));
      }
#pragma unroll
      for (int t = 0; t < 2; ++t) hb.v[t] = hb.v[t] * dtanh(hR.v[t]);
      keep_lds_reads_local();
      PR = to4_group<2>(L + oR + YR::oV1T + (ln.i & 3) * YR::LR + 16 * t0, ln, hb.v);
    }
    ubar = splat4(0.f);
#pragma unroll
    for (int i = 0; i < N; ++i) ubar[0] = __builtin_fmaf(L[oG + i], lam[i], ubar[0]);
    f32x4 v = splat4(0.f);
#pragma unroll
    for (int j = 0; j < N; ++j) {
      float acc = 0.f;
#pragma unroll
      for (int i = 0; i < N; ++i) acc = __builtin_fmaf(L[oJ + i * N + j], lam[i], acc);
#pragma unroll
      for (int k = 0; k < N; ++k) acc = __builtin_fmaf(-S[j][k], Stl[k], acc);
      v[j] = acc;
    }
    float scaleH, unscaleH;
    f32x4 vn;
    f32x4 PH = hnet_hvp_w(L + oH, ln, tp, v, scaleH, unscaleH, vn);
    xch_put_partial(ln.xch + kXP0, ln, PR);
    xch_put_partial(ln.xch + kXP1, ln, PH);
    __syncthreads();
    f32x4 xb = splat4(0.f);
    xb += xch_sum_partials(ln.xch + kXP0, ln) * unscaleR;
    xbar = xb + (xch_sum_partials(ln.xch + kXP1, ln) * scaleH + curv_apply(cv, vn)) * unscaleH;
  }
};

template <int DUMMY = 0>
struct CanonSplit {
  using Base = CanonModel<128, MM_F16X2>;
  static constexpr int N = 4, HID = 128, T = 8, MM = MM_F16X2;
  static constexpr bool SPLIT = true;
  static constexpr int SCR = 0, IMG = Base::IMG, STASH = Base::STASH, TAPE_C = Base::TAPE_C, oH = Base::oH, oC = Base::oC, MI = 1;
  static constexpr bool CURV = true;
  DEV static float Base_Gu(const float* L, int row, f32x4 u) { return Base::Base_Gu(L, row, u); }
  DEV static f32x4 Base_Gt(const float* L, float dpb0, float dpb1) { return Base::Base_Gt(L, dpb0, dpb1); }

  template <bool WANT_H, int TK = TAPE_NONE, int FE = 0>
  DEV static f32x4 f(const float* L, float* scr, Lane ln, f32x4 y, f32x4 u, float& Hval, float* stash = nullptr) {
    static_assert(!WANT_H, "the split-tile kernels are rollout kernels");
    constexpr bool ST = TK != TAPE_NONE, CT = TK == TAPE_MPC;
    keep_lds_reads_local();
    float a = L[oC + 0], b = L[oC + 1], c = L[oC + 2];
    float sn, cs;
    sincos_dev(y[1], sn, cs);
    float bc = b * cs;
    f32x4 z = {y[0], y[1], a * y[2] + bc * y[3], bc * y[2] + c * y[3]};
    HTapeW tp;
    f32x4 P = hnet_grad_w(L + oH, ln, z, tp, []() {});
    xch_put_partial(ln.xch + kXP0, ln, P);
    if (CT) curv_put_w(L + Base::oP, ln, tp);
    if (ST) {
      store_act<2>(stash + 2 * ln.w * 256, ln, tp.a2);
      if (!CT) store_act<2>(stash + T * 256 + 2 * ln.w * 256, ln, tp.q1);
    }
    __syncthreads();
    f32x4 dH = xch_sum_partials(ln.xch + kXP0, ln);
    if (ST && ln.q == 0 && ln.w == 0) PHNN_NT_STORE(dH, reinterpret_cast<f32x4*>(stash + (CT ? 1 : 2) * T * 256) + ln.i);
    if (CT) store_rf(stash + Base::oTapeC, ln, curv_get_w(L + Base::oP, ln));
    float dp0 = (-dH[0] - L[oC + 6] * dH[2]) + Base_Gu(L, 2, u);
    float dp1 = (-dH[1] - L[oC + 7] * dH[3]) + Base_Gu(L, 3, u);
    float det = (a * c - bc * bc) + 1e-6f;
    float mi00 = c / det, mi01 = -bc / det, mi11 = a / det;
    return f32x4{mi00 * z[2] + mi01 * z[3], mi01 * z[2] + mi11 * z[3], mi00 * dp0 + mi01 * dp1,
                 mi01 * dp0 + mi11 * dp1};
  }

  template <bool ST = false, bool WG = false, int INH = -1, int FE = 0>
  DEV static void vjp(const float* L, float* scr, Lane ln, f32x4 y, f32x4 u, f32x4 lam, f32x4& ybar, f32x4& ubar,
                      const float* stash = nullptr, float* rec = nullptr, float Hbar = 0.f) {
    static_assert(!WG, "weight-gradient records come from the whole-tile kernels");
    keep_lds_reads_local();
    const int t0 = 2 * ln.w;
    float a = L[oC + 0], b = L[oC + 1], c = L[oC + 2];
    float sn, cs;
    sincos_dev(y[1], sn, cs);
    float bc = b * cs;
    f32x4 z = {y[0], y[1], a * y[2] + bc * y[3], bc * y[2] + c * y[3]};
    HTapeW tp;
    Curv cv;
    f32x4 dH;
    if (ST) {
      dH = tape_load_dH<T, true>(stash, ln);
      load_act<2>(stash + t0 * 256, ln, tp.a2);
      load_curv(stash + Base::oTapeC, ln, cv);
      using Y = LayH2<128, MM_F16X2>;
      load_vec<2>(tp.a1, L + oH + Y::oB1 + 16 * t0, ln);
      in_layer_mm<2, MM_F16X2, kInHRecomp>(tp.a1, L + oH, Y::oW1f, Y::oW1h, ln, z, t0);
      tanh_pre_w(tp.a1);
    } else {
      f32x4 P = hnet_grad_w<kInHRecomp>(L + oH, ln, z, tp, []() {});
      xch_put_partial(ln.xch + kXP0, ln, P);
      curv_put_w(L + Base::oP, ln, tp);
      __syncthreads();
      dH = xch_sum_partials(ln.xch + kXP0, ln);
      spread_curv(curv_get_w(L + Base::oP, ln), ln, cv);
    }
    float Rd2 = L[oC + 6], Rd3 = L[oC + 7];
    float dp0 = (-dH[0] - Rd2 * dH[2]) + Base_Gu(L, 2, u);
    float dp1 = (-dH[1] - Rd3 * dH[3]) + Base_Gu(L, 3, u);
    float det = (a * c - bc * bc) + 1e-6f;
    float rdet = 1.0f / det;
    float mi00 = c * rdet, mi01 = -bc * rdet, mi11 = a * rdet;
    float pb0 = lam[0] * mi00 + lam[1] * mi01, pb1 = lam[0] * mi01 + lam[1] * mi11;
    float dpb0 = lam[2] * mi00 + lam[3] * mi01, dpb1 = lam[2] * mi01 + lam[3] * mi11;
    float mb00 = lam[0] * z[2] + lam[2] * dp0;
    float mb01 = lam[0] * z[3] + lam[1] * z[2] + lam[2] * dp1 + lam[3] * dp0;
    float mb11 = lam[1] * z[3] + lam[3] * dp1;
    f32x4 v = {-dpb0, -dpb1, -Rd2 * dpb0, -Rd3 * dpb1};
    ubar = Base_Gt(L, dpb0, dpb1);
    float scaleH, unscaleH;
    f32x4 vn;
    f32x4 PH = hnet_hvp_w(L + oH, ln, tp, v, scaleH, unscaleH, vn);
    xch_put_partial(ln.xch + kXP1, ln, PH);
    __syncthreads();
    f32x4 zb = (xch_sum_partials(ln.xch + kXP1, ln) * scaleH + curv_apply(cv, vn)) * unscaleH;
    zb[2] += pb0;
    zb[3] += pb1;
    float bcb = zb[2] * y[3] + zb[3] * y[2];
    float detb = (-(mb00 * c + mb11 * a) + mb01 * bc) * (rdet * rdet);
    bcb += -mb01 * rdet;
    bcb += -2.0f * bc * detb;
    ybar = f32x4{zb[0], zb[1] + bcb * (-b * sn), zb[2] * a + zb[3] * bc, zb[2] * bc + zb[3] * c};
  }
};

template <int N_, int HID_, int MM_ = MM_F32, int ACT_ = ACT_TANH>
struct OdeModel {
  static constexpr int N = N_, HID = HID_, T = HID / 16, LD = HID + 4, LR = HID + 8, MM = MM_, MI = 1, ACT = ACT_;
  static_assert(ACT_ == ACT_TANH || MM_ == MM_F32, "SiLU / ReLU run on the all-f32 kernels");
  static constexpr bool SPLIT = false;
  static constexpr int SCR = 0;
  static constexpr int WF = MM == MM_F16X2 ? HfImg<HID>::FLOATS : HID * LD;
  static constexpr int oW1f = 0;
  static constexpr int oB1 = oW1f + T * 64;
  static constexpr int oW2 = oB1 + HID;
  static constexpr int oB2 = oW2 + WF;
  static constexpr int oW3 = oB2 + HID;
  static constexpr int oB3 = oW3 + WF;
  static constexpr int oW4r = oB3 + HID;
  static constexpr int oB4 = oW4r + 4 * LR;
  static constexpr int oW4f = oB4 + 4;
  static constexpr int oW1T = oW4f + T * 64;
  static constexpr int oSC = oW1T + 4 * LR;
  static constexpr bool WIDE = N + 1 > 4;
  static constexpr int oW1fu = oSC + 4;
  static constexpr int oW1Tu = oW1fu + (WIDE ? T * 64 : 0);
  static constexpr int IMG = oW1Tu + (WIDE ? 4 * LR : 0);
  static_assert(MM != MM_BF16X3, "ODEFunc has an f32 and an f16x2 variant");
  static_assert(N <= 4, "state dimension up to 4");

  struct Tape {
    Act<T> a1, a2, a3;
  };

  DEV static void layer1(const float* L, Lane ln, f32x4 x, float u, Act<T>& a1) {
    f32x4 in = x;
    if (!WIDE) in[N & 3] = u;
    load_vec<T>(a1, L + oB1, ln);
    in_layer<T>(a1, L + oW1f, ln, sel4(in, ln.q));
    if (WIDE) in_layer<T>(a1, L + oW1fu, ln, ln.q == 0 ? u : 0.f);
    if constexpr (ACT == ACT_TANH) tanh_act<T>(a1);
  }

  DEV static void hidden(const float* L, Lane ln, int oW, int oB, float c, const Act<T>& a, Act<T>& o) {
    load_vec<T>(o, L + oB, ln);
    if constexpr (ACT != ACT_TANH) {
      Act<T> act;
      act_of<ACT, T>(a, act);
      sq_fwd<T, T>(o, L + oW, ln, act);
      return;
    }
    if (MM == MM_F16X2) {
      Split2<T> sp;
      split_act_h<T>(a, sp);
      sq_fwd_h<T>(o, L + oW, ln, sp);
#pragma unroll
      for (int t = 0; t < T; ++t)
#pragma unroll
        for (int r = 0; r < 4; ++r) o.v[t][r] = tanh_scaled(o.v[t][r], c);
    } else {
      sq_fwd<T, T>(o, L + oW, ln, a);
      tanh_act<T>(o);
    }
  }

  DEV static void hidden_T(const float* L, Lane ln, int oW, const Act<T>& d, Act<T>& o) {
    zero_act<T>(o);
    if (MM == MM_F16X2) {
      Split2<T> sp;
      split_act_h<T>(d, sp);
      sq_bwd_h<T>(o, L + oW, ln, sp);
    } else {
      sq_bwd<T, T>(o, L + oW, ln, d);
    }
  }

  DEV static f32x4 fwd(const float* L, Lane ln, f32x4 x, float u, Tape& tp) {
    keep_lds_reads_local();
    layer1(L, ln, x, u, tp.a1);
    hidden(L, ln, oW2, oB2, L[oSC + 0], tp.a1, tp.a2);
    hidden(L, ln, oW3, oB3, L[oSC + 1], tp.a2, tp.a3);
    f32x4 b4 = *reinterpret_cast<const f32x4*>(L + oB4);
    if constexpr (ACT != ACT_TANH) {
      Act<T> act;
      act_of<ACT, T>(tp.a3, act);
      return to4_rep<T>(L + oW4r, ln, act) + b4;
    }
    return to4_rep<T>(L + oW4r, ln, tp.a3) + b4;
  }

  static constexpr int VEC24 = ACT == ACT_TANH ? T * 192 : T * 256;
  static constexpr int STASH = 2 * VEC24;
  static constexpr bool CURV = false;

  template <bool WANT_H, int TK = TAPE_NONE, int FE = 0>
  DEV static f32x4 f(const float* L, float* scr, Lane ln, f32x4 x, f32x4 uv, float& Hval, float* stash = nullptr) {
    constexpr bool ST = TK != TAPE_NONE;
    const float u = uv[0];
    Tape tp;
    if (WANT_H) Hval = 0.f;
    f32x4 dx = fwd(L, ln, x, u, tp);
    if (ST) {
      if constexpr (ACT == ACT_TANH) {
        store_act24<T>(stash, ln, tp.a2);
        store_act24<T>(stash + VEC24, ln, tp.a3);
      } else {
        store_act<T>(stash, ln, tp.a2);
        store_act<T>(stash + VEC24, ln, tp.a3);
      }
    }
    return dx;
  }

  template <bool ST = false, bool WG = false, int INH = -1, int FE = 0>
  DEV static void vjp(const float* L, float* scr, Lane ln, f32x4 x, f32x4 uv, f32x4 lam, f32x4& xbar, f32x4& ubar4,
                      const float* stash = nullptr, float* rec = nullptr, float Hbar = 0.f) {
    static_assert(!WG, "ODEFunc has no weight-gradient kernels");
    const float u = uv[0];
    float ubar;
    Tape tp;
    if (ST) {
      if constexpr (ACT == ACT_TANH) {
        load_act24<T>(stash + VEC24, ln, tp.a3);
        load_act24<T>(stash, ln, tp.a2);
      } else {
        load_act<T>(stash + VEC24, ln, tp.a3);
        load_act<T>(stash, ln, tp.a2);
      }
      keep_lds_reads_local();
      layer1(L, ln, x, u, tp.a1);
    } else {
      (void)fwd(L, ln, x, u, tp);
    }
    float unscale = 1.0f;
    if (MM == MM_F16X2) {
      float mx = fmaxf(fmaxf(__builtin_fabsf(lam[0]), __builtin_fabsf(lam[1])), fmaxf(__builtin_fabsf(lam[2]), __builtin_fabsf(lam[3])));
      int e = 0;
      (void)__builtin_frexpf(mx, &e);
      e = (mx > 0.f && mx < 3.0e38f) ? e : 0;
      lam = lam * __builtin_ldexpf(1.0f, -e);
      unscale = __builtin_ldexpf(1.0f, e);
    }
    Act<T> d, e;
    zero_act<T>(d);
    in_layer<T>(d, L + oW4f, ln, sel4(lam, ln.q));
    if constexpr (ACT != ACT_TANH) {
      mul_d1<ACT, T>(d, tp.a3);
      hidden_T(L, ln, oW3, d, e);
      mul_d1<ACT, T>(e, tp.a2);
      hidden_T(L, ln, oW2, e, d);
      mul_d1<ACT, T>(d, tp.a1);
    } else {
#pragma unroll
      for (int t = 0; t < T; ++t) d.v[t] = d.v[t] * dtanh(tp.a3.v[t]);
      hidden_T(L, ln, oW3, d, e);
#pragma unroll
      for (int t = 0; t < T; ++t) e.v[t] = e.v[t] * dtanh(tp.a2.v[t]);
      hidden_T(L, ln, oW2, e, d);
#pragma unroll
      for (int t = 0; t < T; ++t) d.v[t] = d.v[t] * dtanh(tp.a1.v[t]);
    }
    f32x4 inb = to4_rep<T>(L + oW1T, ln, d);
    if (MM == MM_F16X2) inb = inb * unscale;
    if (WIDE) {
      ubar = to4_rep<T>(L + oW1Tu, ln, d)[0] * unscale;
    } else {
      ubar = inb[N & 3];
      inb[N & 3] = 0.f;
    }
    xbar = inb;
    ubar4 = f32x4{ubar, 0.f, 0.f, 0.f};
  }
};

DEV void no_speculation() { asm volatile("" ::: "memory"); }

template <int N, class Tgt>
DEV float state_cost(const phnn_cost& c, f32x4 x, const Tgt& tgt) {
  float e[N], cost = 0.f;
#pragma unroll
  for (int i = 0; i < N; ++i) e[i] = x[i] - tgt[i];
#pragma unroll
  for (int j = 0; j < N; ++j) {
    float s = 0.f;
#pragma unroll
    for (int i = 0; i < N; ++i) s = __builtin_fmaf(e[i], c.Q[i * N + j], s);
    cost = __builtin_fmaf(s, e[j], cost);
  }
  if (c.has_x_min) {
    no_speculation();
    float s = 0.f;
#pragma unroll
    for (int i = 0; i < N; ++i) {
      float v = fmaxf(c.x_min[i] - x[i], 0.f);
      s = __builtin_fmaf(v, v, s);
    }
    cost = __builtin_fmaf(c.barrier_weight, s, cost);
  }
  if (c.has_x_max) {
    no_speculation();
    float s = 0.f;
#pragma unroll
    for (int i = 0; i < N; ++i) {
      float v = fmaxf(x[i] - c.x_max[i], 0.f);
      s = __builtin_fmaf(v, v, s);
    }
    cost = __builtin_fmaf(c.barrier_weight, s, cost);
  }
  return cost;
}

template <int N, class Tgt>
DEV f32x4 state_cost_grad(const phnn_cost& c, const float (&Qs)[16], f32x4 x, const Tgt& tgt) {
  float e[N];
  f32x4 g = splat4(0.f);
#pragma unroll
  for (int i = 0; i < N; ++i) e[i] = x[i] - tgt[i];
#pragma unroll
  for (int i = 0; i < N; ++i) {
    float s = 0.f;
#pragma unroll
    for (int j = 0; j < N; ++j) s = __builtin_fmaf(Qs[i * N + j], e[j], s);
    g[i] = s;
  }
  if (c.has_x_min) {
    no_speculation();
#pragma unroll
    for (int i = 0; i < N; ++i) g[i] = __builtin_fmaf(-2.0f * c.barrier_weight, fmaxf(c.x_min[i] - x[i], 0.f), g[i]);
  }
  if (c.has_x_max) {
    no_speculation();
#pragma unroll
    for (int i = 0; i < N; ++i) g[i] = __builtin_fmaf(2.0f * c.barrier_weight, fmaxf(x[i] - c.x_max[i], 0.f), g[i]);
  }
  return g;
}

struct RollParams {
  const float* img;
  const float* x0;
  const float* u;
  const float* traj_in;
  const float* traj_bar;
  const float* cost_bar;
  float* cost;
  float* traj;
  float* grad_u;
  float* grad_x0;
  float* stash;
  const float* dx_bar;
  float* dx_out;
  float* wrec;
  int no_cost;
  long long B;
  int H;
  float dt, half_dt, sixth_dt;
  phnn_cost c;
  float Qs[16];
  const float* x_ref;
  long long ref_bs, ref_ts;
  int ref_rows;
  const int* ref_off_dev;
  int ref_off_host;
};

struct PointParams {
  const float* img;
  const float* x;
  const float* u;
  const float* lam;
  float* dx;
  float* Hout;
  long long B;
  const float* Hbar;
  float* wrec;
};

template <int IMG>
DEV void stage_image(float* lds, const float* img) {
  const f32x4* src = reinterpret_cast<const f32x4*>(img);
  f32x4* dst = reinterpret_cast<f32x4*>(lds);
  for (int k = threadIdx.x; k < IMG / 4; k += blockDim.x) dst[k] = src[k];
  __syncthreads();
}

template <int N>
DEV f32x4 load_state(const float* p) {
  if (N == 4) return *reinterpret_cast<const f32x4*>(p);
  f32x4 x = splat4(0.f);
#pragma unroll
  for (int i = 0; i < N; ++i) x[i] = p[i];
  return x;
}
template <int N>
DEV void store_state(float* p, f32x4 x) {
// ... 910 lines not shown
```

### phnn_mpc_amd/csrc/phnn_pack.h

```cpp
#pragma once
#include "phnn_variants.h"

#define PK_HD __host__ __device__ inline
#if defined(__HIP_DEVICE_COMPILE__)
#define PK_FOR(k, n) for (int k = (int)threadIdx.x; k < (int)(n); k += (int)blockDim.x)
#define PK_SYNC() __syncthreads()
#else
#define PK_FOR(k, n) for (int k = 0; k < (int)(n); ++k)
#define PK_SYNC() ((void)0)
#endif

constexpr int kPackThreads = 1024;

template <class F>
PK_HD float pk_max(int n, float* red, F f) {
  float m = 0.f;
  PK_FOR(k, n) m = fmaxf(m, f(k));
#if defined(__HIP_DEVICE_COMPILE__)
  red[threadIdx.x] = m;
  __syncthreads();
  for (int s = (int)blockDim.x / 2; s > 0; s >>= 1) {
    if ((int)threadIdx.x < s) red[threadIdx.x] = fmaxf(red[threadIdx.x], red[threadIdx.x + s]);
    __syncthreads();
  }
  m = red[0];
  __syncthreads();
#else
  (void)red;
#endif
  return m;
}

PK_HD int pk_unit_of_pos(int pos) {
  const int s = pos / 32, w = pos % 32, q = w / 8, j = w % 8;
  return 32 * s + (j < 4 ? 4 * q + j : 16 + 4 * q + (j - 4));
}

template <int HID>
PK_HD void pack_in_frag(float* dst, const float* W, int nin, float sc) {
  PK_FOR(e, (HID / 16) * 64) {
    const int nt = e >> 6, lane = e & 63, i = lane & 15, q = lane >> 4;
    dst[e] = q < nin ? W[(size_t)(16 * nt + i) * nin + q] * sc : 0.f;
  }
}
template <int HID>
PK_HD void pack_in_frag_h(float* dstf, const float* W, int nin, float sc) {
  _Float16* dst = reinterpret_cast<_Float16*>(dstf);
  PK_FOR(e, (HID / 16) * 64 * 8) {
    const int j = e & 7, lane = (e >> 3) & 63, nt = e >> 9, i = lane & 15, q = lane >> 4, c = j & 3;
    const float x = (q < 2 && c < nin) ? W[(size_t)(16 * nt + i) * nin + c] * sc : 0.f;
    const _Float16 h = (_Float16)x;
    const _Float16 l = (_Float16)(x - (float)h);
    dst[e] = q == 0 ? h : (q == 1 ? l : (_Float16)0.f);
  }
}
template <int HID>
PK_HD void pack_in_frag_T(float* dst, const float* W, int nout) {
  PK_FOR(e, (HID / 16) * 64) {
    const int nt = e >> 6, lane = e & 63, i = lane & 15, q = lane >> 4;
    dst[e] = q < nout ? W[(size_t)q * HID + 16 * nt + i] : 0.f;
  }
}
PK_HD void pack_rows(float* dst, const float* W, int rows, int cols, int ld, float sc = 1.0f) {
  PK_FOR(e, rows * cols) {
    const int r = e / cols, c = e % cols;
    dst[(size_t)r * ld + c] = W[e] * sc;
  }
}
PK_HD void pack_cols_as_rows(float* dst, const float* W, int rows, int cols, int ld, float div = 1.0f) {
  PK_FOR(e, rows * cols) {
    const int r = e / cols, c = e % cols;
    dst[(size_t)c * ld + r] = W[e] / div;
  }
}
PK_HD void pack_copy(float* dst, const float* src, int n, float sc = 1.0f) {
  PK_FOR(k, n) dst[k] = src[k] * sc;
}

PK_HD uint16_t pk_bf16_rne(float x) {
  const uint32_t u = __builtin_bit_cast(uint32_t, x);
  return (uint16_t)((u + 0x7FFFu + ((u >> 16) & 1u)) >> 16);
}
PK_HD float pk_bf16_to_f32(uint16_t b) { return __builtin_bit_cast(float, ((uint32_t)b) << 16); }

template <int HID>
PK_HD void pack_bf16x3(float* dstf, const float* W, float sc) {
  using I = BfImg<HID>;
  uint16_t* dst = reinterpret_cast<uint16_t*>(dstf);
  PK_FOR(e, HID * HID) {
    const int r = e / HID, pos = e % HID, u = pk_unit_of_pos(pos);
    const float x = W[(size_t)r * HID + u] * sc;
    const uint16_t h = pk_bf16_rne(x);
    const float r1 = x - pk_bf16_to_f32(h);
    const uint16_t m = pk_bf16_rne(r1);
    const uint16_t l = pk_bf16_rne(r1 - pk_bf16_to_f32(m));
    const size_t at = (size_t)r * I::RS + pos;
    dst[at] = h;
    dst[(size_t)I::PART / 2 + at] = m;
    dst[(size_t)I::PART + at] = l;
  }
}

PK_HD float pk_pow2_scale(float mx, bool always) {
  int e = 0;
  if (mx > 0.f && (always || mx < 0.5f || mx >= 1024.0f)) (void)__builtin_frexpf(mx, &e);
  return __builtin_ldexpf(1.0f, -e);
}

template <int HID>
PK_HD float pack_f16x2(float* dstf, const float* W, float sc, float* red) {
  using I = HfImg<HID>;
  const float mx = pk_max(HID * HID, red, [&](int k) { return __builtin_fabsf(W[k] * sc); });
  const float S = pk_pow2_scale(mx, false);
  _Float16* dst = reinterpret_cast<_Float16*>(dstf);
  PK_FOR(e, HID * HID) {
    const int r = e / HID, pos = e % HID, u = pk_unit_of_pos(pos);
    const float x = (W[(size_t)r * HID + u] * sc) * S;
    const _Float16 h = (_Float16)x;
    const _Float16 l = (_Float16)(x - (float)h);
    const size_t at = (size_t)r * I::RS + pos;
    dst[at] = h;
    dst[(size_t)I::PART / 2 + at] = l;
  }
  return S;
}

template <int HID, int MM, bool FOLD = true>
PK_HD const float* pack_h2(float* dst, const float* p, int nin, float* red, float* ssb = nullptr) {
  using Y = LayH2<HID, MM>;
  const float* W1 = p; p += (size_t)HID * nin;
  const float* b1 = p; p += HID;
  const float* W2 = p; p += (size_t)HID * HID;
  const float* b2 = p; p += HID;
  const float* W3 = p; p += HID;
  const float* b3 = p; p += 1;
  const float k1 = (FOLD && kPreScaled<HID / 16>) ? 2.8853900817779268f : 1.0f;
  float S = 1.0f;
  if (MM == MM_BF16X3) pack_bf16x3<HID>(dst + Y::oW2, W2, k1);
  else if (MM == MM_F16X2) S = pack_f16x2<HID>(dst + Y::oW2, W2, k1, red);
  else pack_rows(dst + Y::oW2, W2, HID, HID, Y::LD, k1);
  S *= k1;
  pack_in_frag<HID>(dst + Y::oW1f, W1, nin, k1);
  if (MM == MM_F16X2) pack_in_frag_h<HID>(dst + Y::oW1h, W1, nin, k1);
  pack_copy(dst + Y::oB1, b1, HID, k1);
  pack_copy(dst + Y::oW3, W3, HID);
  float Sb = 1.0f;
  if (MM == MM_F16X2) {
    const float w3max = pk_max(HID, red, [&](int k) { return __builtin_fabsf(W3[k]); });
    const float n1 = pk_max(HID, red, [&](int r) {
      float a = 0.f;
      for (int c = 0; c < nin; ++c) a += __builtin_fabsf(W1[(size_t)r * nin + c]);
      return a;
    });
    const float n2 = pk_max(HID, red, [&](int r) {
      float b = 0.f;
      for (int c = 0; c < HID; ++c) b += __builtin_fabsf(W2[(size_t)r * HID + c]);
      return b;
    });
    const float bound = fmaxf(w3max, 0.77f * w3max * n1 * n2);
    while (bound * Sb > 1024.0f) Sb *= 0.5f;
  }
  PK_FOR(k, HID) {
    dst[Y::oB2 + k] = b2[k] * S;
    dst[Y::oW3B + k] = W3[k] * Sb;
    dst[Y::oW3S + k] = W3[k] * Sb / S;
  }
  if (ssb) *ssb = S * Sb;
  pack_cols_as_rows(dst + Y::oW1T, W1, HID, nin, Y::LR, S * Sb);
  PK_FOR(k, 1) {
    dst[Y::oB3] = b3[0];
    dst[Y::oB3 + 1] = 2.8853900817779268f / S;
    dst[Y::oB3 + 2] = 1.0f / k1;
    dst[Y::oB3 + 3] = Sb;
  }
  return p;
}

template <int HID>
PK_HD void pack_curv(float* dst, const float* W1, int nin, float ssb, float* red) {
  using I = CurvImg<HID>;
  auto pval = [&](int row, int u) {
    int i = 0, r = row;
    while (r >= 4 - i) { r -= 4 - i; ++i; }
    const int j = i + r;
    return j < nin ? W1[(size_t)u * nin + i] * W1[(size_t)u * nin + j] : 0.f;
  };
  const float pmx = pk_max(10 * HID, red, [&](int e) { return __builtin_fabsf(pval(e / HID, e % HID)); });
  const float Sp = pk_pow2_scale(pmx, true);
  _Float16* pw = reinterpret_cast<_Float16*>(dst);
  PK_FOR(e, 10 * HID) {
    const int row = e / HID, pos = e % HID;
    const float x = pval(row, pk_unit_of_pos(pos)) * Sp;
    const _Float16 h = (_Float16)x, l = (_Float16)(x - (float)h);
    pw[(size_t)row * I::RS + pos] = h;
    pw[(size_t)I::PART / 2 + (size_t)row * I::RS + pos] = l;
  }
  PK_FOR(k, 1) dst[I::oConst] = -2.0f / (ssb * Sp);
}

template <int HID, int MM, bool FOLD = true>
PK_HD const float* pack_h1(float* dst, const float* p, int nin, int nout, float* red) {
  using Y = LayH1<HID, MM>;
  const float* V1 = p; p += (size_t)HID * nin;
  const float* c1 = p; p += HID;
  const float* V2 = p; p += (size_t)nout * HID;
  const float* c2 = p; p += nout;
  if (Y::HF) {
    const float mx = pk_max(nout * HID, red, [&](int k) { return __builtin_fabsf(V2[k]); });
    const float Sr = pk_pow2_scale(mx, true);
    _Float16* fw = reinterpret_cast<_Float16*>(dst + Y::oV2);
    _Float16* bw = reinterpret_cast<_Float16*>(dst + Y::oV2T);
    PK_FOR(e, nout * HID) {
      const int o = e / HID, pos = e % HID, u = pk_unit_of_pos(pos);
      const float x = V2[(size_t)o * HID + u] * Sr;
      const _Float16 h = (_Float16)x, l = (_Float16)(x - (float)h);
      fw[(size_t)o * Y::RS + pos] = h;
      fw[(size_t)Y::FPART / 2 + (size_t)o * Y::RS + pos] = l;
      bw[(size_t)u * 16 + o] = h;
      bw[(size_t)Y::BPART / 2 + (size_t)u * 16 + o] = l;
    }
    PK_FOR(k, 1) dst[Y::oSc] = 1.0f / Sr;
  } else {
    pack_rows(dst + Y::oV2, V2, nout, HID, Y::LD);
    PK_FOR(k, 1) dst[Y::oSc] = 1.0f;
  }
  const float k1 = (FOLD && kPreScaled<HID / 16>) ? 2.8853900817779268f : 1.0f;
  pack_in_frag<HID>(dst + Y::oV1f, V1, nin, k1);
  if (Y::HF) pack_in_frag_h<HID>(dst + Y::oV1h, V1, nin, k1);
  pack_copy(dst + Y::oC1, c1, HID, k1);
  pack_copy(dst + Y::oC2, c2, nout);
  pack_cols_as_rows(dst + Y::oV1T, V1, HID, nin, Y::LR);
  return p;
}

PK_HD float pk_softplus(float x) { return x > 20.f ? x : log1pf(expf(x)); }

template <class M>
struct PackOf;

template <int N, int HID, bool FIXG, int MM, int MI, int ACT>
struct PackOf<PhnnModel<N, HID, FIXG, MM, MI, ACT>> {
  using M = PhnnModel<N, HID, FIXG, MM, MI, ACT>;
  PK_HD static void run(float* img, const phnn_desc* d, const float* p, float* red) {
    PK_FOR(k, M::IMG) img[k] = 0.f;
    PK_SYNC();
    const float* J = p; p += N * N;
    const float* G = nullptr;
    if (d->fixed_G) { G = p; p += N * MI; }
    constexpr bool FOLD = ACT == ACT_TANH;
    p = pack_h1<HID, MM, FOLD>(img + M::oR, p, N, N * N, red);
    const float* W1h = p;
    float ssb = 1.0f;
    p = pack_h2<HID, MM, FOLD>(img + M::oH, p, N, red, &ssb);
    if constexpr (M::CURV) pack_curv<HID>(img + M::oP, W1h, N, ssb, red);
    if (!d->fixed_G) p = pack_h1<HID, MM, FOLD>(img + M::oGn, p, N, N * MI, red);
    PK_FOR(e, N * N) {
      const int i = e / N, j = e % N;
      img[M::oJ + e] = J[i * N + j] - J[j * N + i];
    }
    if (G) pack_copy(img + M::oG, G, N * MI);
  }
};

template <int HID, int MM, int MI, int MT, int ACT>
struct PackOf<CanonModel<HID, MM, MI, MT, ACT>> {
  using M = CanonModel<HID, MM, MI, MT, ACT>;
  PK_HD static void run(float* img, const phnn_desc* d, const float* p, float* red) {
    PK_FOR(k, M::IMG) img[k] = 0.f;
    PK_SYNC();
    const float* Rd = p; p += 4;
    const float* G = p; p += 4 * MI;
    float* c = img + M::oC;
    if (MT == MASS_CARTPOLE) {
      const float log_a = p[0], b = p[1], log_c = p[2];
      p += 3;
      PK_FOR(k, 1) {
        c[0] = expf(log_a) + 1e-3f;
        c[1] = b;
        c[2] = expf(log_c) + 1e-3f;
      }
    } else if (MT == MASS_CONSTANT) {
      const float l00 = pk_softplus(p[0]) + 1e-3f, l10 = p[2], l11 = pk_softplus(p[3]) + 1e-3f;
      p += 4;
      const float i00 = 1.0f / l00, i11 = 1.0f / l11, i10 = -l10 / (l00 * l11);
      float* cw = img + M::oCW;
      PK_FOR(k, 1) {
        c[0] = l00 * l00;
        c[1] = l00 * l10;
        c[2] = l10 * l10 + l11 * l11;
        cw[0] = i00 * i00 + i10 * i10;
        cw[1] = i10 * i11;
        cw[2] = i11 * i11;
      }
    } else {
      const int nout = MT == MASS_DIAGONAL ? 2 : 3;
      float* dm = img + M::oMn;
      const float* W1 = p; p += 64 * 2;
      const float* b1 = p; p += 64;
      const float* W2 = p; p += 64 * 64;
      const float* b2 = p; p += 64;
      const float* Wo = p; p += (size_t)nout * 64;
      const float* bo = p; p += nout;
      pack_in_frag<64>(dm + LayM::oW1f, W1, 2, 1.0f);
      pack_copy(dm + LayM::oB1, b1, 64);
      pack_rows(dm + LayM::oW2, W2, 64, 64, LayM::LD);
      pack_copy(dm + LayM::oB2, b2, 64);
      pack_rows(dm + LayM::oWo, Wo, nout, 64, LayM::LR);
      pack_copy(dm + LayM::oBo, bo, nout);
      pack_in_frag_T<64>(dm + LayM::oWoTf, Wo, nout);
      pack_cols_as_rows(dm + LayM::oW1T, W1, 64, 2, LayM::LR);
    }
    const float* W1h = p;
    float ssb = 1.0f;
    p = pack_h2<HID, MM, ACT == ACT_TANH>(img + M::oH, p, 4, red, &ssb);
    if constexpr (M::CURV) pack_curv<HID>(img + M::oP, W1h, 4, ssb, red);
    PK_FOR(i, 4) {
      c[4 + i] = pk_softplus(Rd[i]) + 1e-4f;
      c[8 + i] = Rd[i] > 20.f ? 1.0f : (float)(1.0 / (1.0 + exp(-(double)Rd[i])));
    }
    pack_copy(c + 12, G, 4 * MI);
    (void)d;
  }
};

template <int N, int HID, int MM, int ACT>
struct PackOf<OdeModel<N, HID, MM, ACT>> {
  using M = OdeModel<N, HID, MM, ACT>;
  PK_HD static void run(float* img, const phnn_desc* d, const float* p, float* red) {
    const int nin = N + 1;
    PK_FOR(k, M::IMG) img[k] = 0.f;
    PK_SYNC();
    const float* W1 = p; p += (size_t)HID * nin;
    const float* b1 = p; p += HID;
    const float* W2 = p; p += (size_t)HID * HID;
    const float* b2 = p; p += HID;
    const float* W3 = p; p += (size_t)HID * HID;
    const float* b3 = p; p += HID;
    const float* W4 = p; p += (size_t)N * HID;
    const float* b4 = p; p += N;
    float S2 = 1.0f, S3 = 1.0f;
    pack_in_frag<HID>(img + M::oW1f, W1, nin, 1.0f);
    pack_copy(img + M::oB1, b1, HID);
    if (MM == MM_F16X2) {
      S2 = pack_f16x2<HID>(img + M::oW2, W2, 1.0f, red);
      S3 = pack_f16x2<HID>(img + M::oW3, W3, 1.0f, red);
    } else {
      pack_rows(img + M::oW2, W2, HID, HID, M::LD);
      pack_rows(img + M::oW3, W3, HID, HID, M::LD);
    }
    pack_copy(img + M::oB2, b2, HID, S2);
    pack_copy(img + M::oB3, b3, HID, S3);
    pack_rows(img + M::oW4r, W4, N, HID, M::LR);
    pack_copy(img + M::oB4, b4, N);
    pack_in_frag_T<HID>(img + M::oW4f, W4, N);
    const float S23 = S2 * S3;
    PK_FOR(e, HID * 4) {
      const int r = e >> 2, c = e & 3;
      if (c < nin) img[M::oW1T + (size_t)c * M::LR + r] = W1[(size_t)r * nin + c] / S23;
    }
    if (M::WIDE) {
      PK_FOR(e, (HID / 16) * 16) {
        const int nt = e >> 4, lane = e & 15;
        img[M::oW1fu + nt * 64 + lane] = W1[(size_t)(16 * nt + lane) * nin + N];
      }
      PK_FOR(r, HID) img[M::oW1Tu + r] = W1[(size_t)r * nin + N] / S23;
    }
    PK_FOR(k, 1) {
      img[M::oSC + 0] = 2.8853900817779268f / S2;
      img[M::oSC + 1] = 2.8853900817779268f / S3;
    }
    (void)d;
  }
};

struct PackParams {
  const float* orig;
  const int* pad_src;
  int n_pad;
  float* pblob;
  float* img;
  phnn_desc pdesc;
};
int phnn_pack_launch(int variant, const PackParams& p, hipStream_t st);
```

Measured before the change: 33.11 million.

## Use reciprocal-form tanh derivative and fold layer-2 derivative factors into tape

Adds two derivative-factor variants for the pre-scaled 128-wide f16x2 Tanh MPC kernels, both on by default. One stores g*a in place of a2 so the HVP skips reloading W3S and recomputing 1-a^2. The other recomputes layer-1 activations directly as r-r^2 from the reciprocal, i.e. (1-tanh^2)/4, and compensates with folded scale constants written by the packer. This removes dtanh arithmetic and weight loads in the adjoint, at the cost of extra packed constants, changed numerics and more template complexity.

```diff
diff --git a/phnn_mpc_amd/csrc/phnn_kernels.hip.h b/phnn_mpc_amd/csrc/phnn_kernels.hip.h
--- a/phnn_mpc_amd/csrc/phnn_kernels.hip.h
+++ b/phnn_mpc_amd/csrc/phnn_kernels.hip.h
@@ -117,6 +117,36 @@
     }
 }
 
+#ifndef PHNN_DERIV_SITES
+#define PHNN_DERIV_SITES 3
+#endif
+constexpr bool kDerivE2 = (PHNN_DERIV_SITES & 1) != 0, kDerivRcp = (PHNN_DERIV_SITES & 2) != 0;
+constexpr int kDvE2 = 1, kDvRcp = 2;
+DEV float dtanh_q_pre(float z) {
+  const float r = __builtin_amdgcn_rcpf(__builtin_amdgcn_exp2f(z) + 1.0f);
+  return __builtin_fmaf(-r, r, r);
+}
+template <int T>
+DEV void dtanh_q_act_pre(Act<T>& a) {
+  static_assert(kPreScaled<T>, "the reciprocal form belongs to the pre-scaled (128-wide) images");
+#pragma unroll
+  for (int t = 0; t < T; ++t)
+#pragma unroll
+    for (int r = 0; r < 4; ++r) a.v[t][r] = dtanh_q_pre(a.v[t][r]);
+}
+template <int T>
+DEV void tanh_and_dq_pre(Act<T>& z, Act<T>& a) {
+  static_assert(kPreScaled<T>, "the reciprocal form belongs to the pre-scaled (128-wide) images");
+#pragma unroll
+  for (int t = 0; t < T; ++t)
+#pragma unroll
+    for (int e = 0; e < 4; ++e) {
+      const float r = __builtin_amdgcn_rcpf(__builtin_amdgcn_exp2f(z.v[t][e]) + 1.0f);
+      a.v[t][e] = __builtin_fmaf(-2.0f, r, 1.0f);
+      z.v[t][e] = __builtin_fmaf(-r, r, r);
+    }
+}
+
 template <int T>
 DEV void load_vec(Act<T>& o, const float* vec, Lane ln) {
   keep_lds_reads_local();
@@ -973,8 +1003,9 @@
   return to4_rep<T>(L + Y::oW1T, ln, qd);
 }
 
-template <int HID, bool WANT_H, int MM = MM_F32, int SITE = kInHFwd, int ACT = ACT_TANH, int FE = 0>
+template <int HID, bool WANT_H, int MM = MM_F32, int SITE = kInHFwd, int ACT = ACT_TANH, int FE = 0, bool E2 = false>
 DEV f32x4 hnet_grad(const float* L, Lane ln, f32x4 z, HTape<HID>& tp, float& Hval) {
+  static_assert(!E2 || (MM == MM_F16X2 && ACT == ACT_TANH), "e2 belongs to the f16x2 Tanh MPC kernels");
   if constexpr (ACT != ACT_TANH) {
     static_assert(MM == MM_F32, "SiLU / ReLU run on the all-f32 kernels");
     return hnet_grad_g<HID, WANT_H, ACT>(L, ln, z, tp, Hval);
@@ -1004,9 +1035,9 @@
           const float x = tp.a2.v[t][e + k];
           const float a = decltype(pre)::value ? __builtin_fmaf(-2.0f, __builtin_amdgcn_rcpf(__builtin_amdgcn_exp2f(x) + 1.0f), 1.0f)
                                                : tanh_scaled(x, c);
-          tp.a2.v[t][e + k] = a;
           if (WANT_H) s = __builtin_fmaf(w3[e + k], a, s);
           g[k] = w3b[e + k] * __builtin_fmaf(-a, a, 1.0f);
+          tp.a2.v[t][e + k] = E2 ? g[k] * a : a;
         }
         if (e == 2 && t + 1 < T) {
           if (WANT_H) w3 = *reinterpret_cast<const f32x4*>(L + Y::oW3 + 16 * (t + 1) + 4 * ln.q);
@@ -1054,6 +1085,7 @@
       }
       f32x4 w3b = *reinterpret_cast<const f32x4*>(L + Y::oW3B + 16 * t + 4 * ln.q);
       g.v[t] = w3b * dtanh(tp.a2.v[t]);
+      if constexpr (E2) tp.a2.v[t] = g.v[t] * tp.a2.v[t];
     }
   }
   if (WANT_H) Hval = reduce_q(s) + L[Y::oB3];
@@ -1096,6 +1128,14 @@
   tanh_act_pre<Y::T>(a1);
 }
 
+template <int HID, int MM, int SITE = kInHRecomp>
+DEV void hnet_layer1_dq(const float* L, Lane ln, f32x4 z, Act<HID / 16>& d1) {
+  using Y = LayH2<HID, MM>;
+  load_vec<Y::T>(d1, L + Y::oB1, ln);
+  in_layer_mm<Y::T, MM, SITE>(d1, L, Y::oW1f, Y::oW1h, ln, z);
+  dtanh_q_act_pre<Y::T>(d1);
+}
+
 template <int HID>
 struct CurvImg {
   static constexpr int RS = HID + 16, PART = 10 * RS * 2;
@@ -1184,9 +1224,12 @@
   else load_act<T>(stash + T * 256, ln, tp.q1);
 }
 
-template <int HID, int MM = MM_F32, bool WG = false, int ACT = ACT_TANH, int SITE = kInHHvp, bool CQ = false, int FE = 0>
-DEV f32x4 hnet_hvp(const float* L, Lane ln, HTape<HID>& tp, f32x4 v, float* rec = nullptr, const Curv* cv = nullptr) {
+template <int HID, int MM = MM_F32, bool WG = false, int ACT = ACT_TANH, int SITE = kInHHvp, bool CQ = false, int FE = 0, int DV = 0>
+DEV f32x4 hnet_hvp(const float* L, Lane ln, HTape<HID>& tp, f32x4 v, float* rec = nullptr, const Curv* cv = nullptr,
+                   const float* P = nullptr) {
   static_assert(!CQ || (MM == MM_F16X2 && ACT == ACT_TANH && !WG), "the curvature block exists for f16x2 Tanh MPC kernels");
+  static_assert(DV == 0 || CQ, "derivative factors: the MPC adjoint with the curvature block");
+  constexpr bool E2 = (DV & kDvE2) != 0, DQ = (DV & kDvRcp) != 0;
   if constexpr (ACT != ACT_TANH) {
     static_assert(!WG, "weight-gradient kernels exist for Tanh models only");
     return hnet_hvp_g<HID, ACT>(L, ln, tp, v);
@@ -1199,14 +1242,14 @@
     int e = 0;
     (void)__builtin_frexpf(mx, &e);
     e = (mx > 0.f && mx < 3.0e38f) ? e : 0;
-    v = v * __builtin_ldexpf(1.0f, -e);
-    unscale = __builtin_ldexpf(1.0f, e);
+    v = v * __builtin_ldexpf(DQ ? 4.0f : 1.0f, -e);
+    unscale = __builtin_ldexpf(DQ ? 0.25f : 1.0f, e);
   }
   Act<T> ad1, w;
   zero_act<T>(ad1);
   in_layer_mm<T, MM, SITE>(ad1, L, Y::oW1f, Y::oW1h, ln, v);
 #pragma unroll
-  for (int t = 0; t < T; ++t) ad1.v[t] = dtanh(tp.a1.v[t]) * ad1.v[t];
+  for (int t = 0; t < T; ++t) ad1.v[t] = (DQ ? tp.a1.v[t] : dtanh(tp.a1.v[t])) * ad1.v[t];
   if constexpr (!CQ) {
 #pragma unroll
     for (int t = 0; t < T; ++t) tp.q1.v[t] = tp.q1.v[t] * (tp.a1.v[t] * ad1.v[t]);
@@ -1218,17 +1261,22 @@
   if constexpr (FUSE_ACT) {
     Split2<T> sp;
     split_act_h<T>(ad1, sp);
-    f32x4 w3 = *reinterpret_cast<const f32x4*>(L + Y::oW3S + 4 * ln.q);
+    f32x4 w3 = splat4(0.f);
+    if (!E2) w3 = *reinterpret_cast<const f32x4*>(L + Y::oW3S + 4 * ln.q);
     sq_fwd_h<T>(w, L + Y::oW2, ln, sp, [&](int P, int j) {
       const int t = 2 * P + (j >> 1), e = 2 * (j & 1);
       f32x2 x;
 #pragma unroll
       for (int k = 0; k < 2; ++k) {
         const float a2 = tp.a2.v[t][e + k];
-        const float ad2 = __builtin_fmaf(-a2, a2, 1.0f) * w.v[t][e + k];
-        x[k] = w3[e + k] * (a2 * ad2);
+        if (E2) {
+          x[k] = a2 * w.v[t][e + k];
+        } else {
+          const float ad2 = __builtin_fmaf(-a2, a2, 1.0f) * w.v[t][e + k];
+          x[k] = w3[e + k] * (a2 * ad2);
+        }
       }
-      if (e == 2 && t + 1 < T) w3 = *reinterpret_cast<const f32x4*>(L + Y::oW3S + 16 * (t + 1) + 4 * ln.q);
+      if (!E2 && e == 2 && t + 1 < T) w3 = *reinterpret_cast<const f32x4*>(L + Y::oW3S + 16 * (t + 1) + 4 * ln.q);
       split_put_h<T>(spw, P, j, x);
     });
   } else {
@@ -1246,6 +1294,10 @@
     keep_lds_reads_local();
 #pragma unroll
     for (int t = 0; t < T; ++t) {
+      if constexpr (E2) {
+        w.v[t] = tp.a2.v[t] * w.v[t];
+        continue;
+      }
       f32x4 w3 = *reinterpret_cast<const f32x4*>(L + Y::oW3S + 16 * t + 4 * ln.q);
       f32x4 a2 = tp.a2.v[t];
       f32x4 ad2 = dtanh(a2) * w.v[t];
@@ -1255,6 +1307,10 @@
   }
   Act<T> qd;
   zero_act<T>(qd);
+  float hscale = 0.f;
+  if constexpr (CQ) {
+    hscale = E2 ? P[CurvImg<HID>::oConst + (DQ ? 2 : 1)] : (DQ ? -32.0f : -2.0f) * L[Y::oB3 + 2];
+  }
   if constexpr (FUSABLE) {
     if constexpr (!FUSE_ACT) split_act_h<T>(w, spw);
     if constexpr (FUSE_RED) {
@@ -1262,9 +1318,10 @@
       sq_bwd_h<T>(qd, L + Y::oW2, ln, spw, [&](int P, int j) {
         const int t = 2 * P + (j >> 1), e = 2 * (j & 1);
         const float a0 = tp.a1.v[t][e], a1 = tp.a1.v[t][e + 1];
-        red.put(P, j, qd.v[t][e] * __builtin_fmaf(-a0, a0, 1.0f), qd.v[t][e + 1] * __builtin_fmaf(-a1, a1, 1.0f));
+        if (DQ) red.put(P, j, qd.v[t][e] * a0, qd.v[t][e + 1] * a1);
+        else red.put(P, j, qd.v[t][e] * __builtin_fmaf(-a0, a0, 1.0f), qd.v[t][e + 1] * __builtin_fmaf(-a1, a1, 1.0f));
       });
-      return (red.finish() * (-2.0f * L[Y::oB3 + 2]) + curv_apply(*cv, v)) * unscale;
+      return (red.finish() * hscale + curv_apply(*cv, v)) * unscale;
     } else {
       sq_bwd_h<T>(qd, L + Y::oW2, ln, spw);
     }
@@ -1282,11 +1339,11 @@
   if (WG) store_rec_scaled<T>(rec + 3 * T * 256, ln, qd, unscale);
 #pragma unroll
   for (int t = 0; t < T; ++t) {
-    if constexpr (CQ) qd.v[t] = qd.v[t] * dtanh(tp.a1.v[t]);
+    if constexpr (CQ) qd.v[t] = qd.v[t] * (DQ ? tp.a1.v[t] : dtanh(tp.a1.v[t]));
     else qd.v[t] = __builtin_elementwise_fma(qd.v[t], dtanh(tp.a1.v[t]), tp.q1.v[t]);
   }
   f32x4 Hv = to4_rep<T>(L + Y::oW1T, ln, qd);
-  if constexpr (CQ) return (Hv * (-2.0f * L[Y::oB3 + 2]) + curv_apply(*cv, v)) * unscale;
+  if constexpr (CQ) return (Hv * hscale + curv_apply(*cv, v)) * unscale;
   return Hv * (-2.0f * unscale * L[Y::oB3 + 2]);
 }
 
@@ -1310,7 +1367,7 @@
   return ((o0 + o1) + o2) * inv + c2;
 }
 
-template <int HID, int MM>
+template <int HID, int MM, bool DQ = false>
 DEV void h1_bwd_operands(const float* L, Lane ln, const float (&obar)[16], f16x8& b1, f16x8& b2, float& unscale) {
   using Y = LayH1<HID, MM>;
   float mx = 0.f;
@@ -1320,7 +1377,7 @@
   (void)__builtin_frexpf(mx, &e);
   e = (mx > 0.f && mx < 3.0e38f) ? e : 0;
   const float sc = __builtin_ldexpf(1.0f, -e);
-  unscale = __builtin_ldexpf(1.0f, e) * L[Y::oSc];
+  unscale = __builtin_ldexpf(1.0f, e) * L[Y::oSc + (DQ ? 1 : 0)];
   const bool second = (ln.q & 1) != 0, lo_half = ln.q >= 2;
   u32x4 B1, B2;
 #pragma unroll
@@ -1348,16 +1405,21 @@
     for (int e = 0; e < 4; ++e) rf[4 * k + e] = v[e];
   }
 }
-template <int HID, int MM = MM_F32, int SITE = kInHNet1, int ACT = ACT_TANH>
+template <int HID, int MM = MM_F32, int SITE = kInHNet1, int ACT = ACT_TANH, bool DQ = false>
 DEV void h1_hidden(const float* L, Lane ln, f32x4 x, Act<HID / 16>& h) {
   using Y = LayH1<HID, MM>;
   constexpr int T = Y::T;
   load_vec<T>(h, L + Y::oC1, ln);
   in_layer_mm<T, MM, SITE>(h, L, Y::oV1f, Y::oV1h, ln, x);
+  if constexpr (DQ) {
+    static_assert(ACT == ACT_TANH && Y::HF, "derivative factors: f16x2 Tanh");
+    dtanh_q_act_pre<T>(h);
+    return;
+  }
   if constexpr (ACT == ACT_TANH) tanh_act_pre<T>(h);
 }
 
-template <int HID, int MM = MM_F32, int SITE = kInHNet1, int ACT = ACT_TANH>
+template <int HID, int MM = MM_F32, int SITE = kInHNet1, int ACT = ACT_TANH, bool DQ = false>
 DEV void h1_fwd(const float* L, float* scr, Lane ln, f32x4 x, Act<HID / 16>& h, float (&out)[16], float* rf_stash = nullptr) {
   using Y = LayH1<HID, MM>;
   constexpr int T = Y::T;
@@ -1374,8 +1436,19 @@
     gather16(scr, ln, og.v[0], out);
     return;
   }
+  Act<1> o;
+  if constexpr (DQ) {
+    static_assert(Y::HF, "derivative factors: f16x2 Tanh");
+    Act<T> a;
+    tanh_and_dq_pre<T>(h, a);
+    Split2<T> sp;
+    split_act_h<T>(a, sp);
+    o.v[0] = h1_out_hf<HID, MM>(L, ln, sp);
+    if (rf_stash) store_rf(rf_stash, ln, o.v[0]);
+    gather16(scr, ln, o.v[0], out);
+    return;
+  }
   tanh_act_pre<T>(h);
-  Act<1> o;
   if (Y::HF) {
     Split2<T> sp;
     split_act_h<T>(h, sp);
@@ -1388,10 +1461,11 @@
   gather16(scr, ln, o.v[0], out);
 }
 
-template <int HID, int MM = MM_F32, bool WG = false, int ACT = ACT_TANH>
+template <int HID, int MM = MM_F32, bool WG = false, int ACT = ACT_TANH, bool DQ = false>
 DEV f32x4 h1_bwd(const float* L, Lane ln, const Act<HID / 16>& h, const float (&obar)[16], float* rec = nullptr) {
   using Y = LayH1<HID, MM>;
   constexpr int T = Y::T;
+  static_assert(!DQ || (Y::HF && ACT == ACT_TANH && !WG), "derivative factors: f16x2 Tanh MPC adjoint");
   Act<T> hb;
   if constexpr (ACT != ACT_TANH) {
     static_assert(MM == MM_F32 && !WG, "SiLU / ReLU: all-f32 kernels, no weight-gradient records");
@@ -1407,7 +1481,7 @@
   float unscale = 1.0f;
   if (Y::HF) {
     f16x8 b1, b2;
-    h1_bwd_operands<HID, MM>(L, ln, obar, b1, b2, unscale);
+    h1_bwd_operands<HID, MM, DQ>(L, ln, obar, b1, b2, unscale);
     keep_lds_reads_local();
     const char* base = reinterpret_cast<const char*>(L + Y::oV2T) + ln.i * 32 + (ln.q & 1) * 16;
 #pragma unroll
@@ -1425,7 +1499,7 @@
     sq_bwd<T, 1>(hb, L + Y::oV2, ln, ob);
   }
 #pragma unroll
-  for (int t = 0; t < T; ++t) hb.v[t] = hb.v[t] * dtanh(h.v[t]);
+  for (int t = 0; t < T; ++t) hb.v[t] = hb.v[t] * (DQ ? h.v[t] : dtanh(h.v[t]));
   if (WG) store_rec_scaled<T>(rec, ln, hb, Y::HF ? unscale : 1.0f);
   f32x4 xb = to4_rep<T>(L + Y::oV1T, ln, hb);
   return Y::HF ? xb * unscale : xb;
@@ -1472,6 +1546,8 @@
   static constexpr bool CURV = MM == MM_F16X2 && ACT == ACT_TANH &&
                                4 * (oP + CurvImg<HID>::FLOATS + kMaxWaves * SCR) <= 160 * 1024;
   static constexpr int IMG = oP + (CURV ? CurvImg<HID>::FLOATS : 0);
+  static constexpr bool DERIV = CURV && kPreScaled<T>;
+  static constexpr int DV = DERIV ? (kDerivE2 ? kDvE2 : 0) | (kDerivRcp ? kDvRcp : 0) : 0;
   static constexpr int FUSE = (HID_ != 128 || !FIXG_) ? 0 : ((MI_ <= 2 ? PHNN_FUSE_K1 : 0) | (MI_ == 1 ? PHNN_FUSE_K2 : 0));
 
   static constexpr int oStashRf = 2 * T * 256 + 64;
@@ -1483,7 +1559,7 @@
     constexpr bool ST = TK != TAPE_NONE, CT = TK == TAPE_MPC && CURV;
     keep_lds_reads_local();
     HTape<HID> tp;
-    f32x4 dH = hnet_grad<HID, WANT_H, MM, kInHFwd, ACT, FE>(L + oH, ln, x, tp, Hval);
+    f32x4 dH = hnet_grad<HID, WANT_H, MM, kInHFwd, ACT, FE, CT && (DV & kDvE2) != 0>(L + oH, ln, x, tp, Hval);
     if (ST) hnet_tape_store<HID, CT>(stash, oTapeC, L + oP, ln, tp, dH);
     Act<T> hR;
     float rf[16];
@@ -1540,6 +1616,8 @@
   DEV static void vjp(const float* L, float* scr, Lane ln, f32x4 x, f32x4 u, f32x4 lam, f32x4& xbar, f32x4& ubar,
                       const float* stash = nullptr, float* rec = nullptr, float Hbar = 0.f) {
     constexpr bool CQ = CURV && !WG;
+    constexpr int DQV = CQ ? DV : 0;
+    constexpr bool E2 = (DQV & kDvE2) != 0, DQ = (DQV & kDvRcp) != 0;
     keep_lds_reads_local();
     HTape<HID> tp;
     Curv cv;
@@ -1551,7 +1629,7 @@
       load_rf(stash + (CQ ? oTapeRf : oStashRf), ln, rf);
       hnet_tape_load<HID, CQ>(stash, oTapeC, ln, tp, cv);
     } else {
-      dH = hnet_grad<HID, false, MM, INH & kInHRecomp, ACT>(L + oH, ln, x, tp, Hdummy);
+      dH = hnet_grad<HID, false, MM, INH & kInHRecomp, ACT, 0, E2>(L + oH, ln, x, tp, Hdummy);
       if constexpr (CQ) spread_curv(hnet_curv<HID>(L + oP, ln, tp), ln, cv);
     }
     if (WG && !ST) {
@@ -1563,9 +1641,9 @@
     {
       Act<T> hR;
       if (ST) {
-        h1_hidden<HID, MM, INH & kInHNet1Adj, ACT>(L + oR, ln, x, hR);
+        h1_hidden<HID, MM, INH & kInHNet1Adj, ACT, DQ>(L + oR, ln, x, hR);
       } else {
-        h1_fwd<HID, MM, INH & kInHNet1Adj, ACT>(L + oR, scr, ln, x, hR, rf);
+        h1_fwd<HID, MM, INH & kInHNet1Adj, ACT, DQ>(L + oR, scr, ln, x, hR, rf);
       }
       sym_from_rf<N>(rf, S);
 #pragma unroll
@@ -1581,7 +1659,7 @@
       }
       float rbar[16];
       rbar_from<N>(lam, dH, Stl, StdH, rbar);
-      xb += h1_bwd<HID, MM, WG && RECHB, ACT>(L + oR, ln, hR, rbar, WG && RECHB ? rec + 4 * Rec::VEC : nullptr);
+      xb += h1_bwd<HID, MM, WG && RECHB, ACT, DQ>(L + oR, ln, hR, rbar, WG && RECHB ? rec + 4 * Rec::VEC : nullptr);
       if (WG && ln.q == 0) {
         f32x4* sm = reinterpret_cast<f32x4*>(rec + Rec::oSmall + ln.i * kRecSmall);
 #pragma unroll
@@ -1628,8 +1706,9 @@
       sm[8] = u;
       sm[9] = f32x4{Hbar, 0.f, 0.f, 0.f};
     }
-    if (ST) hnet_layer1<HID, MM, ACT>(L + oH, ln, x, tp.a1);
-    xbar = xb + hnet_hvp<HID, MM, WG, ACT, INH & kInHHvp, CQ, ST ? FE : 0>(L + oH, ln, tp, v, rec, &cv);
+    if constexpr (DQ) hnet_layer1_dq<HID, MM, (ST ? -1 : INH) & kInHRecomp>(L + oH, ln, x, tp.a1);
+    else if (ST) hnet_layer1<HID, MM, ACT>(L + oH, ln, x, tp.a1);
+    xbar = xb + hnet_hvp<HID, MM, WG, ACT, INH & kInHHvp, CQ, ST ? FE : 0, DQV>(L + oH, ln, tp, v, rec, &cv, L + oP);
     if (WG) xbar = xbar + Hbar * dH;
   }
 };
@@ -1725,6 +1804,8 @@
   static constexpr int oMn = oC + 32;
   static constexpr int oP = oMn + (MT_ >= MASS_DIAGONAL ? LayM::SIZE : 0);
   static constexpr bool CURV = MM_ == MM_F16X2 && ACT_ == ACT_TANH;
+  static constexpr bool DERIV = CURV && kPreScaled<T>;
+  static constexpr int DV = DERIV ? (kDerivE2 ? kDvE2 : 0) | (kDerivRcp ? kDvRcp : 0) : 0;
   static constexpr int FUSE = (HID_ == 128 && MT_ <= MASS_CONSTANT) ? PHNN_FUSE_K1 : 0;
   static constexpr int IMG = oP + (CURV ? CurvImg<HID>::FLOATS : 0);
 
@@ -1764,7 +1845,7 @@
       mass_eval(L, ln, y, m, w, mt);
       f32x4 z = {y[0], y[1], m[0] * y[2] + m[1] * y[3], m[1] * y[2] + m[2] * y[3]};
       HTape<HID> tp;
-      f32x4 dH = hnet_grad<HID, WANT_H, MM, kInHFwd, ACT, FE>(L + oH, ln, z, tp, Hval);
+      f32x4 dH = hnet_grad<HID, WANT_H, MM, kInHFwd, ACT, FE, CT && (DV & kDvE2) != 0>(L + oH, ln, z, tp, Hval);
       if (ST) hnet_tape_store<HID, CT>(stash, oTapeC, L + oP, ln, tp, dH);
       float dp0 = (-dH[0] - L[oC + 6] * dH[2]) + Base_Gu(L, 2, u);
       float dp1 = (-dH[1] - L[oC + 7] * dH[3]) + Base_Gu(L, 3, u);
@@ -1776,7 +1857,7 @@
     float bc = b * cs;
     f32x4 z = {y[0], y[1], a * y[2] + bc * y[3], bc * y[2] + c * y[3]};
     HTape<HID> tp;
-    f32x4 dH = hnet_grad<HID, WANT_H, MM, kInHFwd, ACT, FE>(L + oH, ln, z, tp, Hval);
+    f32x4 dH = hnet_grad<HID, WANT_H, MM, kInHFwd, ACT, FE, CT && (DV & kDvE2) != 0>(L + oH, ln, z, tp, Hval);
     if (ST) hnet_tape_store<HID, CT>(stash, oTapeC, L + oP, ln, tp, dH);
     float dp0 = (-dH[0] - L[oC + 6] * dH[2]) + Base_Gu(L, 2, u);
     float dp1 = (-dH[1] - L[oC + 7] * dH[3]) + Base_Gu(L, 3, u);
@@ -1793,6 +1874,8 @@
   DEV static void vjp(const float* L, float* scr, Lane ln, f32x4 y, f32x4 u, f32x4 lam, f32x4& ybar, f32x4& ubar,
                       const float* stash = nullptr, float* rec = nullptr, float Hbar = 0.f) {
     constexpr bool CQ = CURV && !WG;
+    constexpr int DQV = CQ ? DV : 0;
+    constexpr bool E2 = (DQV & kDvE2) != 0, DQ = (DQV & kDvRcp) != 0;
     Curv cv;
     keep_lds_reads_local();
     if constexpr (MT != MASS_CARTPOLE) {
@@ -1806,10 +1889,12 @@
       if (ST) {
         dH = tape_load_dH<T, CQ>(stash, ln);
         hnet_tape_load<HID, CQ>(stash, oTapeC, ln, tp, cv);
-        hnet_layer1<HID, MM, ACT>(L + oH, ln, z, tp.a1);
+        if constexpr (DQ) hnet_layer1_dq<HID, MM>(L + oH, ln, z, tp.a1);
+        else hnet_layer1<HID, MM, ACT>(L + oH, ln, z, tp.a1);
       } else {
-        dH = hnet_grad<HID, false, MM, INH & kInHRecomp, ACT>(L + oH, ln, z, tp, Hdummy);
+        dH = hnet_grad<HID, false, MM, INH & kInHRecomp, ACT, 0, E2>(L + oH, ln, z, tp, Hdummy);
         if constexpr (CQ) spread_curv(hnet_curv<HID>(L + oP, ln, tp), ln, cv);
+        if constexpr (DQ) hnet_layer1_dq<HID, MM, INH & kInHRecomp>(L + oH, ln, z, tp.a1);
       }
       const float Rd2 = L[oC + 6], Rd3 = L[oC + 7];
       const float dp0 = (-dH[0] - Rd2 * dH[2]) + Base_Gu(L, 2, u);
@@ -1834,7 +1919,7 @@
           sm[9] = f32x4{Hbar, 0.f, 0.f, 0.f};
         }
       }
-      f32x4 zb = hnet_hvp<HID, MM, WG, ACT, INH & kInHHvp, CQ, ST ? FE : 0>(L + oH, ln, tp, v, rec, &cv);
+      f32x4 zb = hnet_hvp<HID, MM, WG, ACT, INH & kInHHvp, CQ, ST ? FE : 0, DQV>(L + oH, ln, tp, v, rec, &cv, L + oP);
       if (WG) zb = zb + Hbar * dH;
       zb[2] += pb0;
       zb[3] += pb1;
@@ -1876,10 +1961,12 @@
     if (ST) {
       dH = tape_load_dH<T, CQ>(stash, ln);
       hnet_tape_load<HID, CQ>(stash, oTapeC, ln, tp, cv);
-      hnet_layer1<HID, MM, ACT>(L + oH, ln, z, tp.a1);
+      if constexpr (DQ) hnet_layer1_dq<HID, MM>(L + oH, ln, z, tp.a1);
+      else hnet_layer1<HID, MM, ACT>(L + oH, ln, z, tp.a1);
     } else {
-      dH = hnet_grad<HID, false, MM, INH & kInHRecomp, ACT>(L + oH, ln, z, tp, Hdummy);
+      dH = hnet_grad<HID, false, MM, INH & kInHRecomp, ACT, 0, E2>(L + oH, ln, z, tp, Hdummy);
       if constexpr (CQ) spread_curv(hnet_curv<HID>(L + oP, ln, tp), ln, cv);
+      if constexpr (DQ) hnet_layer1_dq<HID, MM, INH & kInHRecomp>(L + oH, ln, z, tp.a1);
     }
     float Rd2 = L[oC + 6], Rd3 = L[oC + 7];
     float dp0 = (-dH[0] - Rd2 * dH[2]) + Base_Gu(L, 2, u);
@@ -1910,7 +1997,7 @@
         sm[9] = f32x4{Hbar, 0.f, 0.f, 0.f};
       }
     }
-    f32x4 zb = hnet_hvp<HID, MM, WG, ACT, INH & kInHHvp, CQ, ST ? FE : 0>(L + oH, ln, tp, v, rec, &cv);
+    f32x4 zb = hnet_hvp<HID, MM, WG, ACT, INH & kInHHvp, CQ, ST ? FE : 0, DQV>(L + oH, ln, tp, v, rec, &cv, L + oP);
     if (WG) zb = zb + Hbar * dH;
     zb[2] += pb0;
     zb[3] += pb1;
@@ -1944,6 +2031,12 @@
   return to4_kslots(((p[0] + p[64]) + p[128]) + p[192]);
 }
 
+DEV void dtanh_q_pre_w(ActW& a) {
+#pragma unroll
+  for (int t = 0; t < 2; ++t)
+#pragma unroll
+    for (int r = 0; r < 4; ++r) a.v[t][r] = dtanh_q_pre(a.v[t][r]);
+}
 DEV void tanh_pre_w(ActW& a) {
 #pragma unroll
   for (int t = 0; t < 2; ++t)
@@ -2006,7 +2099,7 @@
   return (((p[0] + p[64]) + p[128]) + p[192]) * P[CurvImg<128>::oConst];
 }
 
-template <int SITE = kInHFwd, class PreBarrier>
+template <int SITE = kInHFwd, bool E2 = false, class PreBarrier>
 DEV f32x4 hnet_grad_w(const float* L, Lane ln, f32x4 z, HTapeW& tp, PreBarrier pre_barrier) {
   using Y = LayH2<128, MM_F16X2>;
   const int t0 = 2 * ln.w;
@@ -2041,6 +2134,7 @@
   for (int t = 0; t < 2; ++t) {
     f32x4 w3b = *reinterpret_cast<const f32x4*>(L + Y::oW3B + 16 * (t0 + t) + 4 * ln.q);
     g.v[t] = w3b * dtanh(tp.a2.v[t]);
+    if constexpr (E2) tp.a2.v[t] = g.v[t] * tp.a2.v[t];
   }
   {
     Split2<2> sp;
@@ -2060,21 +2154,30 @@
   return to4_group<2>(L + Y::oW1T + (ln.i & 3) * Y::LR + 16 * t0, ln, g.v);
 }
 
-DEV f32x4 hnet_hvp_w(const float* L, Lane ln, HTapeW& tp, f32x4 v, float& scale, float& unscale, f32x4& vn) {
+template <int SITE = kInHRecomp>
+DEV void hnet_layer1_dq_w(const float* L, Lane ln, f32x4 z, ActW& d1) {
+  using Y = LayH2<128, MM_F16X2>;
+  const int t0 = 2 * ln.w;
+  load_vec<2>(d1, L + Y::oB1 + 16 * t0, ln);
+  in_layer_mm<2, MM_F16X2, SITE>(d1, L, Y::oW1f, Y::oW1h, ln, z, t0);
+  dtanh_q_pre_w(d1);
+}
+
+DEV f32x4 hnet_hvp_w(const float* L, const float* P, Lane ln, HTapeW& tp, f32x4 v, float& scale, float& unscale, f32x4& vn) {
   using Y = LayH2<128, MM_F16X2>;
   const int t0 = 2 * ln.w;
   float mx = fmaxf(fmaxf(__builtin_fabsf(v[0]), __builtin_fabsf(v[1])), fmaxf(__builtin_fabsf(v[2]), __builtin_fabsf(v[3])));
   int e = 0;
   (void)__builtin_frexpf(mx, &e);
   e = (mx > 0.f && mx < 3.0e38f) ? e : 0;
-  v = v * __builtin_ldexpf(1.0f, -e);
+  v = v * __builtin_ldexpf(kDerivRcp ? 4.0f : 1.0f, -e);
   vn = v;
-  unscale = __builtin_ldexpf(1.0f, e);
+  unscale = __builtin_ldexpf(kDerivRcp ? 0.25f : 1.0f, e);
   ActW ad1, w;
   zero_act<2>(ad1);
   in_layer_mm<2, MM_F16X2, kInHHvp>(ad1, L, Y::oW1f, Y::oW1h, ln, v, t0);
 #pragma unroll
-  for (int t = 0; t < 2; ++t) ad1.v[t] = dtanh(tp.a1.v[t]) * ad1.v[t];
+  for (int t = 0; t < 2; ++t) ad1.v[t] = (kDerivRcp ? tp.a1.v[t] : dtanh(tp.a1.v[t])) * ad1.v[t];
   {
     Split2<2> sp;
     split_act_h<2>(ad1, sp);
@@ -2090,6 +2193,10 @@
   keep_lds_reads_local();
 #pragma unroll
   for (int t = 0; t < 2; ++t) {
+    if constexpr (kDerivE2) {
+      w.v[t] = tp.a2.v[t] * w.v[t];
+      continue;
+    }
     f32x4 w3 = *reinterpret_cast<const f32x4*>(L + Y::oW3S + 16 * (t0 + t) + 4 * ln.q);
     f32x4 a2 = tp.a2.v[t];
     f32x4 ad2 = dtanh(a2) * w.v[t];
@@ -2109,8 +2216,8 @@
     sq_bwd_h_w(qd, L + Y::oW2, ln, all);
   }
 #pragma unroll
-  for (int t = 0; t < 2; ++t) qd.v[t] = qd.v[t] * dtanh(tp.a1.v[t]);
-  scale = -2.0f * L[Y::oB3 + 2];
+  for (int t = 0; t < 2; ++t) qd.v[t] = qd.v[t] * (kDerivRcp ? tp.a1.v[t] : dtanh(tp.a1.v[t]));
+  scale = kDerivE2 ? P[CurvImg<128>::oConst + (kDerivRcp ? 2 : 1)] : (kDerivRcp ? -32.0f : -2.0f) * L[Y::oB3 + 2];
   keep_lds_reads_local();
   return to4_group<2>(L + Y::oW1T + (ln.i & 3) * Y::LR + 16 * t0, ln, qd.v);
 }
@@ -2125,18 +2232,35 @@
   static constexpr int oH = Base::oH, oR = Base::oR, oJ = Base::oJ, oG = Base::oG;
   using YR = LayH1<128, MM_F16X2>;
 
-  template <int SITE = kInHNet1>
+  template <int SITE = kInHNet1, bool DQ = false>
   DEV static void rnet_hidden(const float* L, Lane ln, f32x4 x, ActW& hR) {
     const int t0 = 2 * ln.w;
     load_vec<2>(hR, L + oR + YR::oC1 + 16 * t0, ln);
     in_layer_mm<2, MM_F16X2, SITE>(hR, L + oR, YR::oV1f, YR::oV1h, ln, x, t0);
-    tanh_pre_w(hR);
-  }
-  template <int SITE = kInHNet1>
+    if (DQ) dtanh_q_pre_w(hR);
+    else tanh_pre_w(hR);
+  }
+  template <int SITE = kInHNet1, bool DQ = false>
   DEV static void rnet_layer1(const float* L, Lane ln, f32x4 x, ActW& hR) {
-    rnet_hidden<SITE>(L, ln, x, hR);
     Split2<2> sp;
-    split_act_h<2>(hR, sp);
+    if constexpr (DQ) {
+      const int t0 = 2 * ln.w;
+      load_vec<2>(hR, L + oR + YR::oC1 + 16 * t0, ln);
+      in_layer_mm<2, MM_F16X2, SITE>(hR, L + oR, YR::oV1f, YR::oV1h, ln, x, t0);
+      ActW a;
+#pragma unroll
+      for (int t = 0; t < 2; ++t)
+#pragma unroll
+        for (int e = 0; e < 4; ++e) {
+          const float r = __builtin_amdgcn_rcpf(__builtin_amdgcn_exp2f(hR.v[t][e]) + 1.0f);
+          a.v[t][e] = __builtin_fmaf(-2.0f, r, 1.0f);
+          hR.v[t][e] = __builtin_fmaf(-r, r, r);
+        }
+      split_act_h<2>(a, sp);
+    } else {
+      rnet_hidden<SITE>(L, ln, x, hR);
+      split_act_h<2>(hR, sp);
+    }
     xch_put(ln.xch + kXR2, ln, sp);
   }
   DEV static void rnet_out(const float* L, float* scr, Lane ln, float (&rf)[16], float* rf_stash = nullptr) {
@@ -2154,7 +2278,7 @@
     keep_lds_reads_local();
     HTapeW tp;
     ActW hR;
-    f32x4 P = hnet_grad_w(L + oH, ln, x, tp, [&]() { rnet_layer1(L, ln, x, hR); });
+    f32x4 P = hnet_grad_w<kInHFwd, CT && kDerivE2>(L + oH, ln, x, tp, [&]() { rnet_layer1(L, ln, x, hR); });
     xch_put_partial(ln.xch + kXP0, ln, P);
     if (CT) curv_put_w(L + Base::oP, ln, tp);
     float rf[16];
@@ -2192,12 +2316,14 @@
       using Y = LayH2<128, MM_F16X2>;
       load_vec<2>(tp.a1, L + oH + Y::oB1 + 16 * t0, ln);
       in_layer_mm<2, MM_F16X2, kInHRecomp>(tp.a1, L + oH, Y::oW1f, Y::oW1h, ln, x, t0);
-      tanh_pre_w(tp.a1);
-      rnet_hidden<kInHNet1Adj>(L, ln, x, hR);
+      if (kDerivRcp) dtanh_q_pre_w(tp.a1);
+      else tanh_pre_w(tp.a1);
+      rnet_hidden<kInHNet1Adj, kDerivRcp>(L, ln, x, hR);
     } else {
-      f32x4 P = hnet_grad_w<kInHRecomp>(L + oH, ln, x, tp, [&]() { rnet_layer1<kInHNet1Adj>(L, ln, x, hR); });
+      f32x4 P = hnet_grad_w<kInHRecomp, kDerivE2>(L + oH, ln, x, tp, [&]() { rnet_layer1<kInHNet1Adj, kDerivRcp>(L, ln, x, hR); });
       xch_put_partial(ln.xch + kXP0, ln, P);
       curv_put_w(L + Base::oP, ln, tp);
+      if (kDerivRcp) hnet_layer1_dq_w(L + oH, ln, x, tp.a1);
       rnet_out(L, scr, ln, rf);
       __syncthreads();
       dH = xch_sum_partials(ln.xch + kXP0, ln);
@@ -2222,7 +2348,7 @@
     f32x4 PR;
     {
       f16x8 b1, b2;
-      h1_bwd_operands<128, MM_F16X2>(L + oR, ln, rbar, b1, b2, unscaleR);
+      h1_bwd_operands<128, MM_F16X2, kDerivRcp>(L + oR, ln, rbar, b1, b2, unscaleR);
       keep_lds_reads_local();
       const char* base = reinterpret_cast<const char*>(L + oR + YR::oV2T) + ln.i * 32 + (ln.q & 1) * 16;
       ActW hb;
@@ -2233,7 +2359,7 @@
         hb.v[t] = mfma_h(ah, b1, mfma_h(al, b2, splat4(0.f)));
       }
 #pragma unroll
-      for (int t = 0; t < 2; ++t) hb.v[t] = hb.v[t] * dtanh(hR.v[t]);
+      for (int t = 0; t < 2; ++t) hb.v[t] = hb.v[t] * (kDerivRcp ? hR.v[t] : dtanh(hR.v[t]));
       keep_lds_reads_local();
       PR = to4_group<2>(L + oR + YR::oV1T + (ln.i & 3) * YR::LR + 16 * t0, ln, hb.v);
     }
@@ -2252,7 +2378,7 @@
     }
     float scaleH, unscaleH;
     f32x4 vn;
-    f32x4 PH = hnet_hvp_w(L + oH, ln, tp, v, scaleH, unscaleH, vn);
+    f32x4 PH = hnet_hvp_w(L + oH, L + Base::oP, ln, tp, v, scaleH, unscaleH, vn);
     xch_put_partial(ln.xch + kXP0, ln, PR);
     xch_put_partial(ln.xch + kXP1, ln, PH);
     __syncthreads();
@@ -2283,7 +2409,7 @@
     float bc = b * cs;
     f32x4 z = {y[0], y[1], a * y[2] + bc * y[3], bc * y[2] + c * y[3]};
     HTapeW tp;
-    f32x4 P = hnet_grad_w(L + oH, ln, z, tp, []() {});
+    f32x4 P = hnet_grad_w<kInHFwd, CT && kDerivE2>(L + oH, ln, z, tp, []() {});
     xch_put_partial(ln.xch + kXP0, ln, P);
     if (CT) curv_put_w(L + Base::oP, ln, tp);
     if (ST) {
@@ -2323,11 +2449,13 @@
       using Y = LayH2<128, MM_F16X2>;
       load_vec<2>(tp.a1, L + oH + Y::oB1 + 16 * t0, ln);
       in_layer_mm<2, MM_F16X2, kInHRecomp>(tp.a1, L + oH, Y::oW1f, Y::oW1h, ln, z, t0);
-      tanh_pre_w(tp.a1);
+      if (kDerivRcp) dtanh_q_pre_w(tp.a1);
+      else tanh_pre_w(tp.a1);
     } else {
-      f32x4 P = hnet_grad_w<kInHRecomp>(L + oH, ln, z, tp, []() {});
+      f32x4 P = hnet_grad_w<kInHRecomp, kDerivE2>(L + oH, ln, z, tp, []() {});
       xch_put_partial(ln.xch + kXP0, ln, P);
       curv_put_w(L + Base::oP, ln, tp);
+      if (kDerivRcp) hnet_layer1_dq_w(L + oH, ln, z, tp.a1);
       __syncthreads();
       dH = xch_sum_partials(ln.xch + kXP0, ln);
       spread_curv(curv_get_w(L + Base::oP, ln), ln, cv);
@@ -2347,7 +2475,7 @@
     ubar = Base_Gt(L, dpb0, dpb1);
     float scaleH, unscaleH;
     f32x4 vn;
-    f32x4 PH = hnet_hvp_w(L + oH, ln, tp, v, scaleH, unscaleH, vn);
+    f32x4 PH = hnet_hvp_w(L + oH, L + Base::oP, ln, tp, v, scaleH, unscaleH, vn);
     xch_put_partial(ln.xch + kXP1, ln, PH);
     __syncthreads();
     f32x4 zb = (xch_sum_partials(ln.xch + kXP1, ln) * scaleH + curv_apply(cv, vn)) * unscaleH;
diff --git a/phnn_mpc_amd/csrc/phnn_pack.h b/phnn_mpc_amd/csrc/phnn_pack.h
--- a/phnn_mpc_amd/csrc/phnn_pack.h
+++ b/phnn_mpc_amd/csrc/phnn_pack.h
@@ -126,7 +126,7 @@
 }
 
 template <int HID, int MM, bool FOLD = true>
-PK_HD const float* pack_h2(float* dst, const float* p, int nin, float* red, float* ssb = nullptr) {
+PK_HD const float* pack_h2(float* dst, const float* p, int nin, float* red, float* ssb = nullptr, float* k1s = nullptr) {
   using Y = LayH2<HID, MM>;
   const float* W1 = p; p += (size_t)HID * nin;
   const float* b1 = p; p += HID;
@@ -166,6 +166,7 @@
     dst[Y::oW3S + k] = W3[k] * Sb / S;
   }
   if (ssb) *ssb = S * Sb;
+  if (k1s) *k1s = k1 * S;
   pack_cols_as_rows(dst + Y::oW1T, W1, HID, nin, Y::LR, S * Sb);
   PK_FOR(k, 1) {
     dst[Y::oB3] = b3[0];
@@ -177,7 +178,7 @@
 }
 
 template <int HID>
-PK_HD void pack_curv(float* dst, const float* W1, int nin, float ssb, float* red) {
+PK_HD void pack_curv(float* dst, const float* W1, int nin, float ssb, float k1s, float* red) {
   using I = CurvImg<HID>;
   auto pval = [&](int row, int u) {
     int i = 0, r = row;
@@ -195,7 +196,11 @@
     pw[(size_t)row * I::RS + pos] = h;
     pw[(size_t)I::PART / 2 + (size_t)row * I::RS + pos] = l;
   }
-  PK_FOR(k, 1) dst[I::oConst] = -2.0f / (ssb * Sp);
+  PK_FOR(k, 1) {
+    dst[I::oConst] = -2.0f / (ssb * Sp);
+    dst[I::oConst + 1] = -2.0f / k1s;
+    dst[I::oConst + 2] = 16.0f * (-2.0f / k1s);
+  }
 }
 
 template <int HID, int MM, bool FOLD = true>
@@ -219,7 +224,10 @@
       bw[(size_t)u * 16 + o] = h;
       bw[(size_t)Y::BPART / 2 + (size_t)u * 16 + o] = l;
     }
-    PK_FOR(k, 1) dst[Y::oSc] = 1.0f / Sr;
+    PK_FOR(k, 1) {
+      dst[Y::oSc] = 1.0f / Sr;
+      dst[Y::oSc + 1] = 4.0f / Sr;
+    }
   } else {
     pack_rows(dst + Y::oV2, V2, nout, HID, Y::LD);
     PK_FOR(k, 1) dst[Y::oSc] = 1.0f;
@@ -250,9 +258,9 @@
     constexpr bool FOLD = ACT == ACT_TANH;
     p = pack_h1<HID, MM, FOLD>(img + M::oR, p, N, N * N, red);
     const float* W1h = p;
-    float ssb = 1.0f;
-    p = pack_h2<HID, MM, FOLD>(img + M::oH, p, N, red, &ssb);
-    if constexpr (M::CURV) pack_curv<HID>(img + M::oP, W1h, N, ssb, red);
+    float ssb = 1.0f, k1s = 1.0f;
+    p = pack_h2<HID, MM, FOLD>(img + M::oH, p, N, red, &ssb, &k1s);
+    if constexpr (M::CURV) pack_curv<HID>(img + M::oP, W1h, N, ssb, k1s, red);
     if (!d->fixed_G) p = pack_h1<HID, MM, FOLD>(img + M::oGn, p, N, N * MI, red);
     PK_FOR(e, N * N) {
       const int i = e / N, j = e % N;
@@ -311,9 +319,9 @@
       pack_cols_as_rows(dm + LayM::oW1T, W1, 64, 2, LayM::LR);
     }
     const float* W1h = p;
-    float ssb = 1.0f;
-    p = pack_h2<HID, MM, ACT == ACT_TANH>(img + M::oH, p, 4, red, &ssb);
-    if constexpr (M::CURV) pack_curv<HID>(img + M::oP, W1h, 4, ssb, red);
+    float ssb = 1.0f, k1s = 1.0f;
+    p = pack_h2<HID, MM, ACT == ACT_TANH>(img + M::oH, p, 4, red, &ssb, &k1s);
+    if constexpr (M::CURV) pack_curv<HID>(img + M::oP, W1h, 4, ssb, k1s, red);
     PK_FOR(i, 4) {
       c[4 + i] = pk_softplus(Rd[i]) + 1e-4f;
       c[8 + i] = Rd[i] > 20.f ? 1.0f : (float)(1.0 / (1.0 + exp(-(double)Rd[i])));
```

After: 33.43 million, median of 6. About the same (+1.0%).
